# HyeonwooNoh/RAU_VQA

Measured on AMD Instinct MI355X. Metric: QA-pairs/sec fwd+bwd, Ours_SS 8-step RAU, batch 256, 14x14x512, higher is better.
Workload: dtype f32; 1 GPU; Ours_SS 8-step RAU fwd+bwd, 14x14x512, configs[1]; batch_per_gpu=256, global_batch=256, T=26, feature_map=14x14x512, hops=8, parallelism=dp1, collective=none, hop_weights=SS (x nHop), arithmetic=f32 operands, f32 MFMA accumulate, dropout=train mode, Philox masks per step and rank, launch=eager, 3 streams

## Files before the change

### rau_vqa_amd/csrc/gemm_conv.hip

```cpp
#include <cstdlib>

#include "gemm_core.h"
#include "kernels.h"

namespace rau {

constexpr int BK = 32;



static bool wide_on(int which) {
  static const int mask = [] { const char* e = std::getenv("RAU_CONV_WIDE"); return e ? std::atoi(e) : 3; }();
  return (mask & which) != 0;
}
static int wide_per_cu() {
  static const int v = [] { const char* e = std::getenv("RAU_CONV_WIDE_PER_CU"); return e ? std::atoi(e) : 1; }();
  return v == 2 ? 2 : 1;
}

hipError_t conv_embed_fwd(hipStream_t st, int nB, int D, int S, int M, const float* X,
                          const float* WiT, const float* bi, float* I, int bf16, int one_per_cu) {
  GemmParams P{};
  P.M = M; P.N = nB * S; P.K = D; P.nk = (D + BK - 1) / BK;
  P.A = WiT; P.a_rs = M;
  P.B = X; P.b_rs = S; P.b_bs = (long)D * S;
  P.S = S;
  P.C = I; P.c_bs = (long)M * S;
  P.bias = bi;
  P.act = 1;
  if (!bf16 && wide_on(1) && conv_wide_ok(M, D, S, M) && nB >= 4) {
    const int n4 = nB & ~3;
    hipError_t e = conv_wide(st, 0, n4, M, D, S, WiT, M, X, (long)D * S, I, (long)M * S, bi, 1, nullptr,
                             nullptr, nullptr, nullptr, 0, one_per_cu ? 1 : wide_per_cu());
    if (e != hipSuccess || n4 == nB) return e;
    return conv_embed_fwd(st, nB - n4, D, S, M, X + (size_t)n4 * D * S, WiT, bi, I + (size_t)n4 * M * S,
                          bf16, one_per_cu);
  }
  if (!bf16 && conv_sample_ok(S, 1))
    return conv_sample(st, 0, nB, M, D, S, WiT, M, X, (long)D * S, I, (long)M * S, bi, 1, nullptr, nullptr);
  if (bf16 == 2) return launch_gemm<128, 128, BK, SRC_RC, SRC_RC_FLAT, EPI_CONV, 2>(st, P, 1);
  if (bf16) return launch_gemm<128, 128, BK, SRC_RC, SRC_RC_FLAT, EPI_CONV, 1>(st, P, 1);
  return launch_gemm<128, 128, BK, SRC_RC, SRC_RC_FLAT, EPI_CONV>(st, P, 1, one_per_cu ? 30 * 1024 : 0);
}

static int b16_fwd_pad() { return 1024; }
hipError_t conv_embed_fwd_b16(hipStream_t st, int nB, int D, int S, int M, const void* X16,
                              const void* WiT16, const float* bi, float* I) {
  GemmParams P{};
  P.M = M; P.N = nB * S; P.K = D; P.nk = (D + BK - 1) / BK;
  P.A = reinterpret_cast<const float*>(WiT16); P.a_rs = M;
  P.B = reinterpret_cast<const float*>(X16); P.b_rs = S; P.b_bs = (long)D * S;
  P.S = S;
  P.C = I; P.c_bs = (long)M * S;
  P.bias = bi;
  P.act = 1;
  return launch_gemm<128, 128, BK, SRC_RC_B16, SRC_RC_FLAT_B16, EPI_CONV, 1>(st, P, 1, b16_fwd_pad());
}
hipError_t conv_att_pre_b16(hipStream_t st, int nB, int M, int S, int A, const float* I,
                            const void* WpT16, const float* bp, float* Pout) {
  GemmParams P{};
  P.M = A; P.N = nB * S; P.K = M; P.nk = (M + BK - 1) / BK;
  P.A = reinterpret_cast<const float*>(WpT16); P.a_rs = A;
  P.B = I; P.b_rs = S; P.b_bs = (long)M * S;
  P.S = S;
  P.C = Pout; P.c_bs = (long)A * S;
  P.bias = bp;
  P.act = 0;
  return launch_gemm<128, 128, BK, SRC_RC_B16, SRC_RC_FLAT, EPI_CONV, 1>(st, P, 1, b16_fwd_pad());
}

hipError_t conv_att_pre(hipStream_t st, int nB, int M, int S, int A, const float* I,
                        const float* WpT, const float* bp, float* Pout, int bf16, int one_per_cu) {
  GemmParams P{};
  P.M = A; P.N = nB * S; P.K = M; P.nk = (M + BK - 1) / BK;
  P.A = WpT; P.a_rs = A;
  P.B = I; P.b_rs = S; P.b_bs = (long)M * S;
  P.S = S;
  P.C = Pout; P.c_bs = (long)A * S;
  P.bias = bp;
  P.act = 0;
  if (!bf16 && wide_on(2) && conv_wide_ok(A, M, S, A) && nB >= 4) {
    const int n4 = nB & ~3;
    hipError_t e = conv_wide(st, 0, n4, A, M, S, WpT, A, I, (long)M * S, Pout, (long)A * S, bp, 0, nullptr,
                             nullptr, nullptr, nullptr, 0, one_per_cu ? 1 : wide_per_cu());
    if (e != hipSuccess || n4 == nB) return e;
    return conv_att_pre(st, nB - n4, M, S, A, I + (size_t)n4 * M * S, WpT, bp, Pout + (size_t)n4 * A * S,
                        bf16, one_per_cu);
  }
  if (!bf16 && conv_sample_ok(S, 2))
    return conv_sample(st, 0, nB, A, M, S, WpT, A, I, (long)M * S, Pout, (long)A * S, bp, 0, nullptr, nullptr);
  if (bf16 == 2) return launch_gemm<128, 128, BK, SRC_RC, SRC_RC_FLAT, EPI_CONV, 2>(st, P, 1);
  if (bf16) return launch_gemm<128, 128, BK, SRC_RC, SRC_RC_FLAT, EPI_CONV, 1>(st, P, 1);
  return launch_gemm<128, 128, BK, SRC_RC, SRC_RC_FLAT, EPI_CONV>(st, P, 1, one_per_cu ? 30 * 1024 : 0);
}

hipError_t conv_att_dgrad(hipStream_t st, int nB, int M, int S, int A, const float* dS,
                          const float* Wp, const float* dj, const float* a, float* dI, int bf16) {
  GemmParams P{};
  P.M = M; P.N = nB * S; P.K = A; P.nk = (A + BK - 1) / BK;
  P.A = Wp; P.a_rs = M;
  P.B = dS; P.b_rs = S; P.b_bs = (long)A * S;
  P.S = S;
  P.C = dI; P.c_bs = (long)M * S;
  P.v1 = dj; P.v2 = a;
  if (bf16 != 2 && M % 4 == 0 && conv_sample_ok(S, 4))
    return conv_sample(st, 1, nB, M, A, S, Wp, M, dS, (long)A * S, dI, (long)M * S, nullptr, 0, dj, a);
  if (bf16 == 2) return launch_gemm<128, 128, BK, SRC_RC, SRC_RC_FLAT, EPI_OUTER, 2>(st, P, 1);
  if (bf16) return launch_gemm<128, 128, BK, SRC_RC, SRC_RC_FLAT, EPI_OUTER, 1>(st, P, 1);
  return launch_gemm<128, 128, BK, SRC_RC, SRC_RC_FLAT, EPI_OUTER>(st, P, 1);
}

bool conv_dz_fused_ok(int S, int M, int bf16) {
  return bf16 != 2 && M % 4 == 0 && conv_sample_ok(S, 4);
}
hipError_t conv_att_dgrad_dz(hipStream_t st, int nB, int M, int S, int A, const float* dS,
                             const float* Wp, const float* dj, const float* a, const float* I,
                             float* dZ, float* rs, int dz16, int bf16, int ds16, int light) {
  if (bf16 == 1 && dgrad16_ok(M, A, S, M))
    return dgrad16(st, nB, M, A, S, Wp, M, dS, (long)A * S, dZ, (long)M * S, dj, a, I, rs, dz16, ds16);
  if (ds16) return hipErrorInvalidValue;
  if (!dz16 && !light && dgrad_dma_ok(M, A, S, M))
    return dgrad_dma(st, nB, M, A, S, Wp, M, dS, (long)A * S, dZ, (long)M * S, dj, a, I, rs);
  return conv_sample(st, 2, nB, M, A, S, Wp, M, dS, (long)A * S, dZ, (long)M * S, nullptr, 0, dj, a, I, rs,
                     dz16);
}

hipError_t conv_embed_dgrad(hipStream_t st, int nB, int D, int S, int M, const float* dZ,
                            const float* Wi, float* dX) {
  GemmParams P{};
  P.M = D; P.N = nB * S; P.K = M; P.nk = (M + BK - 1) / BK;
  P.A = Wi; P.a_rs = D;
  P.B = dZ; P.b_rs = S; P.b_bs = (long)M * S;
  P.S = S;
  P.C = dX; P.c_bs = (long)D * S;
  P.bias = nullptr;
  P.act = 0;
  if (conv_sample_ok(S, 8))
    return conv_sample(st, 0, nB, D, M, S, Wi, D, dZ, (long)M * S, dX, (long)D * S, nullptr, 0, nullptr, nullptr);
  return launch_gemm<128, 128, BK, SRC_RC, SRC_RC_FLAT, EPI_CONV>(st, P, 1);
}

static int conv_wgrad_splits(int nB, int rowsA, int rowsB) {
  const int tiles = ((rowsA + 127) / 128) * ((rowsB + 127) / 128);
  constexpr int target = 512;
  int s = target / tiles;
  if (s > nB) s = nB;
  if (s < 1) s = 1;
  return s;
}
size_t conv_wgrad_slab_floats(int nB, int rowsA, int rowsB, int S) {
  return (size_t)conv_wgrad_splits(nB, rowsA, rowsB) * ((size_t)rowsA * rowsB + rowsA);
}

template <int BKT, int ASRC, int DT = 0, int BSRC = SRC_SC>
static hipError_t conv_wgrad(hipStream_t st, GemmParams P, int nB, int S, float* dW,
                             float* slab, float* drow = nullptr) {
  P.S = S;
  P.cps = (S + BKT - 1) / BKT;
  P.K = S;
  P.nk = nB * P.cps;
  const int s = conv_wgrad_splits(nB, P.M, P.N);
  const int spb = (nB + s - 1) / s;
  P.C = slab; P.c_rs = P.N; P.slab_stride = (long)P.M * P.N;
  P.tiles_m = (P.M + 127) / 128;
  P.tiles_n = (P.N + 127) / 128;
  P.nk_per_split = spb * P.cps;
  const int splits = (P.nk + P.nk_per_split - 1) / P.nk_per_split;
  P.rs_out = drow ? slab + (size_t)splits * P.M * P.N : nullptr;
  {
    dim3 grid(8 * ((splits + 7) / 8) * P.tiles_m * P.tiles_n);
    hipLaunchKernelGGL((gemm_split_xcd_kernel<128, 128, BKT, ASRC, BSRC, EPI_SLAB, DT>), grid,
                       dim3(256), 0, st, P, splits);
  }
  hipError_t e = hipGetLastError();
  if (e != hipSuccess) return e;
  e = splitk_reduce_acc(st, (size_t)P.M * P.N, splits, slab, (size_t)P.M * P.N, dW);
  if (e != hipSuccess || !drow) return e;
  return splitk_reduce_acc(st, (size_t)P.M, splits, P.rs_out, (size_t)P.M, drow);
}
template <int ASRC>
static hipError_t conv_wgrad_any(hipStream_t st, const GemmParams& P, int nB, int S, float* dW,
                                 float* slab, int bf16, float* drow = nullptr) {
  if (!bf16 && ASRC == SRC_SC && !drow && wgrad_dma_ok(P.M, P.N, S))
    return wgrad_dma(st, nB, P.M, P.N, S, P.A, P.a_bs, P.B, P.b_bs, dW, slab, conv_wgrad_splits(nB, P.M, P.N));
  if (bf16 == 2) return conv_wgrad<32, ASRC, 2>(st, P, nB, S, dW, slab, drow);
  if (bf16) return conv_wgrad<32, ASRC, 1>(st, P, nB, S, dW, slab, drow);
  if (S % 28 == 0) return conv_wgrad<28, ASRC>(st, P, nB, S, dW, slab, drow);
  return conv_wgrad<32, ASRC>(st, P, nB, S, dW, slab, drow);
}

hipError_t conv_att_wgrad(hipStream_t st, int nB, int M, int S, int A, const float* dS,
                          const float* I, float* dWp, float* slab, int bf16) {
  GemmParams P{};
  P.M = A; P.N = M;
  P.A = dS; P.a_bs = (long)A * S;
  P.B = I; P.b_bs = (long)M * S;
  return conv_wgrad_any<SRC_SC>(st, P, nB, S, dWp, slab, bf16);
}

hipError_t conv_att_wgrad_ds16(hipStream_t st, int nB, int M, int S, int A, const void* dS16,
                               const float* I, float* dWp, float* slab) {
  GemmParams P{};
  P.M = A; P.N = M;
  P.A = reinterpret_cast<const float*>(dS16); P.a_bs = (long)A * S;
  P.B = I; P.b_bs = (long)M * S;
  return conv_wgrad<32, SRC_SC_B16, 1, SRC_SC>(st, P, nB, S, dWp, slab);
}

hipError_t conv_embed_wgrad(hipStream_t st, int nB, int D, int S, int M, const float* dI,
                            const float* I, const float* X, float* dWi, float* slab, int bf16,
                            float* dbi, int dz_final) {
  GemmParams P{};
  P.M = M; P.N = D;
  P.A = dI; P.A2 = I; P.a_bs = (long)M * S;
  P.B = X; P.b_bs = (long)D * S;
  if (dz_final) return conv_wgrad_any<SRC_SC>(st, P, nB, S, dWi, slab, bf16);
  return conv_wgrad_any<SRC_SC_DTANH>(st, P, nB, S, dWi, slab, bf16, dbi);
}

hipError_t conv_embed_wgrad_b16(hipStream_t st, int nB, int D, int S, int M, const void* dZ16,
                                const void* X16, float* dWi, float* slab) {
  if (wgrad16_ok(M, D, S))
    return wgrad16(st, nB, M, D, S, dZ16, (long)M * S, X16, (long)D * S, dWi, slab);
  GemmParams P{};
  P.M = M; P.N = D;
  P.A = reinterpret_cast<const float*>(dZ16); P.a_bs = (long)M * S;
  P.B = reinterpret_cast<const float*>(X16); P.b_bs = (long)D * S;
  return conv_wgrad<32, SRC_SC_B16, 1, SRC_SC_B16>(st, P, nB, S, dWi, slab);
}

}
```

### rau_vqa_amd/csrc/kernels.h

```cpp
#pragma once
#include <hip/hip_runtime.h>
#include <stddef.h>
#include <stdint.h>

#include "../../include/rau.h"

namespace rau {

constexpr long kMaxSplits = 4096;
constexpr hipError_t kSplitStateError = hipErrorIllegalState;
void split_ws_register(const float* base, size_t floats);
void split_ws_unregister(const float* base);
bool split_span_ok(const float* slab, long nsplit, size_t per_split_floats);

struct LinOpts {
  const float* bias = nullptr;
  const float* bias2 = nullptr;
  const float* addend = nullptr;
  long add_rs = 0;
  int accumulate = 0;
  int act = 0;
  const float* ymul = nullptr;
  long y_rs = 0;
  const uint32_t* emask = nullptr;
  size_t emask_e0 = 0;
  float emscale = 1.f;
  float alpha = 1.f;
  float* slab = nullptr;
  size_t slab_floats = 0;
  int* defer_splits = nullptr;
};
hipError_t gemm_nt(hipStream_t st, int M, int N, int K, const float* A, long lda,
                   const float* W, long ldw, float* C, long ldc, const LinOpts& o);
hipError_t gemm_nn(hipStream_t st, int M, int N, int K, const float* A, long lda,
                   const float* W, long ldw, float* C, long ldc, const LinOpts& o);
hipError_t gemm_nt_batched_deferred(hipStream_t st, int nb, int M, int N, int K,
                                    const float* const* A, long lda, const float* const* W,
                                    long ldw, float* slab, size_t slab_floats, int* splits);
hipError_t gemm_nn_batched_deferred(hipStream_t st, int nb, int M, int N, int K,
                                    const float* const* A, long lda, const float* const* W,
                                    long ldw, float* slab, size_t slab_floats, int* splits);
hipError_t gemm_nt_hetero_deferred(hipStream_t st, int nb, int M, int K, const float* A, long lda,
                                   const float* const* W, long ldw, const int* N, float* slab,
                                   size_t slab_floats, int* splits, size_t* off);
size_t gemm_tn_slab_floats(int M, int N, int K);
hipError_t gemm_tn_acc(hipStream_t st, int M, int N, int K, const float* A, long lda,
                       const float* B, long ldb, float* C, long ldc, float* slab,
                       float* dbias = nullptr, int bf16 = 0);

struct TnProblem {
  int M, N; const float* A; long lda; const float* B; long ldb; float* C; float* dbias;
};
size_t gemm_tn_group_slab_floats(const TnProblem* pr, int np, int K);
hipError_t gemm_tn_group_acc(hipStream_t st, const TnProblem* pr, int np, int K, float* slab,
                             size_t slab_floats, int bf16 = 0);

hipError_t conv_embed_fwd(hipStream_t st, int nB, int D, int S, int M, const float* X,
                          const float* WiT , const float* bi, float* I, int bf16 = 0,
                          int one_per_cu = 0 );
hipError_t conv_embed_fwd_b16(hipStream_t st, int nB, int D, int S, int M, const void* X16,
                              const void* WiT16, const float* bi, float* I);
hipError_t conv_att_pre_b16(hipStream_t st, int nB, int M, int S, int A, const float* I,
                            const void* WpT16, const float* bp, float* Pout);
hipError_t conv_att_pre(hipStream_t st, int nB, int M, int S, int A, const float* I,
                        const float* WpT , const float* bp, float* P, int bf16 = 0,
                        int one_per_cu = 0);
bool conv_sample_ok(int S, int which);
hipError_t conv_sample(hipStream_t st, int epi, int nB, int M, int K, int S, const float* Wt,
                       long w_rs, const float* X, long x_bs, float* C, long c_bs,
                       const float* bias, int act, const float* dj, const float* av,
                       const float* Y = nullptr, float* rs = nullptr, int c16 = 0);
bool conv_wide_ok(int M, int K, int S, long w_rs);
hipError_t conv_wide(hipStream_t st, int epi, int nB, int M, int K, int S, const float* Wt, long w_rs,
                     const float* X, long x_bs, float* C, long c_bs, const float* bias, int act,
                     const float* dj, const float* av, const float* Y, float* rs, int c16, int per_cu);
hipError_t transpose2d(hipStream_t st, int rows, int cols, const float* in, float* out,
                       void* out16 = nullptr);
hipError_t conv_att_dgrad(hipStream_t st, int nB, int M, int S, int A, const float* dS,
                          const float* Wp, const float* dj, const float* a, float* dI,
                          int bf16 = 0);
bool conv_dz_fused_ok(int S, int M, int bf16);
hipError_t conv_att_dgrad_dz(hipStream_t st, int nB, int M, int S, int A, const float* dS,
                             const float* Wp, const float* dj, const float* a, const float* I,
                             float* dZ, float* rs, int dz16 = 0,
                             int bf16 = 0,
                             int ds16 = 0,
                             int light = 0);
bool dgrad16_ok(int M, int K, int S, long w_rs);
hipError_t dgrad16(hipStream_t st, int nB, int M, int K, int S, const float* Wt, long w_rs,
                   const void* X, long x_bs, void* C, long c_bs, const float* dj, const float* av,
                   const float* Y, float* rs, int c16, int x16 = 0 );
bool dgrad_dma_ok(int M, int K, int S, long w_rs);
hipError_t dgrad_dma(hipStream_t st, int nB, int M, int K, int S, const float* Wt, long w_rs,
                     const float* X, long x_bs, float* C, long c_bs, const float* dj, const float* av,
                     const float* Y, float* rs);
hipError_t conv_att_wgrad_ds16(hipStream_t st, int nB, int M, int S, int A, const void* dS16,
                               const float* I, float* dWp, float* slab);
hipError_t conv_embed_dgrad(hipStream_t st, int nB, int D, int S, int M, const float* dZ,
                            const float* Wi, float* dX);
size_t conv_wgrad_slab_floats(int nB, int rowsA, int rowsB, int S);
bool wgrad16_ok(int ra, int rb, int S);
size_t wgrad16_slab_floats(int nB, int ra, int rb, int S);
hipError_t wgrad16(hipStream_t st, int nB, int ra, int rb, int S, const void* A16, long a_bs,
                   const void* B16, long b_bs, float* dW, float* slab);
bool skinny_dma_ok(int M, int K, long lda, long ldb, bool brc, int nprob, const int* N,
                   const float* const* A, const float* const* B);
int skinny_dma_splits(int M, int K, int tiles_all, size_t cols_all, size_t slab_floats);
void skinny_dma_set_deep(int on);
void lin_set_bf16(int on);
int lin_bf16();
hipError_t skinny_dma(hipStream_t st, bool brc, int nprob, int M, int K, const float* const* A,
                      long lda, const float* const* B, long ldb, const int* N, float* slab,
                      const long* off, int splits);
bool wgrad_dma_ok(int ra, int rb, int S);
hipError_t wgrad_dma(hipStream_t st, int nB, int ra, int rb, int S, const float* A, long a_bs,
                     const float* B, long b_bs, float* dW, float* slab, int splits);
hipError_t conv_att_wgrad(hipStream_t st, int nB, int M, int S, int A, const float* dS,
                          const float* I, float* dWp, float* slab, int bf16 = 0);
hipError_t conv_embed_wgrad(hipStream_t st, int nB, int D, int S, int M, const float* dI,
                            const float* I, const float* X, float* dWi, float* slab,
                            int bf16 = 0, float* dbi = nullptr ,
                            int dz_final = 0 );
hipError_t conv_embed_wgrad_b16(hipStream_t st, int nB, int D, int S, int M, const void* dZ16,
                                const void* X16, float* dWi, float* slab);

enum GateOrder { GATES_ATT = 0 ,
                 GATES_DEEP = 1  };

hipError_t fill_masks(hipStream_t st, uint64_t seed, uint32_t site, uint32_t step, float p,
                      size_t n, uint32_t* bits, const uint64_t* key_dev = nullptr);
hipError_t embed_fwd(hipStream_t st, int rows, int E, int V, const float* emb, const int32_t* tokens,
                     const uint32_t* mask, float mscale, float* we, size_t mask_e0 = 0);
hipError_t embed_bwd_rows(hipStream_t st, int rows, int E, int V, const int32_t* tokens, const float* dwe,
                          const float* we, const uint32_t* mask, size_t mask_e0, float mscale,
                          float* gE);
hipError_t lstm_fwd(hipStream_t st, int order, int nB, int R, float* g4, const float* c_prev,
                    long cp_rs, float* c, long c_rs, float* h, long h_rs, float* tanhc,
                    float* drop_out, const uint32_t* mask, size_t mask_e0, float mscale,
                    const float* slab = nullptr, int nsplit = 0);
hipError_t lstm_bwd(hipStream_t st, int order, int nB, int R, const float* gates,
                    const float* c_prev, long cp_rs, const float* tanhc, const float* dh,
                    long dh_rs, const float* dh2, const float* dc_next, float* dsum,
                    float* dc_prev, const int32_t* lens, int t, const float* dq_c,
                    const float* dq_h, long dq_rs, const float* slab = nullptr, int nsplit = 0);
struct LstmFwdCell {
  float* g4;
  int has_input;
  const float* b1; const float* b2;
  const float* slab; int nsplit;
  const float* c_prev; long cp_rs;
  float* c; long c_rs; float* h; long h_rs; float* tanhc;
  float* drop_out; const uint32_t* mask; size_t mask_e0; float mscale;
};
struct LstmFwdCells { int n; LstmFwdCell c[2]; };
hipError_t lstm_fwd_multi(hipStream_t st, int order, int nB, int R, const LstmFwdCells& cells);
struct EncWsParams {
  int B, R, TL, P;
  float *G1, *G2, *h1, *c1, *tc1, *x2, *h2, *c2, *tc2;
  const float *Wh1, *Wi2, *Wh2, *bi2, *bh2;
  const uint32_t* mask; float mscale;
  unsigned* cnt; int* err;
  int bf16 = 0;
};
bool enc_ws_ok(int B, int R);
int enc_ws_workgroups(int B);
bool enc_ws_coresident(int B, int blocks_per_cu, int n_cus);
bool enc_ws_fits_device(int B);
hipError_t enc_ws_forward(hipStream_t st, int order, EncWsParams Q);
struct LstmBwdCell {
  const float* gates; const float* c_prev; long cp_rs; const float* tanhc;
  const float* slabA; int nA;
  const float* slabB; int nBp;
  const uint32_t* maskB; size_t maskB_e0; float mscaleB;
  const float* dc_next; float* dsum; float* dc_prev;
  int t; const float* dq_c; const float* dq_h;
};
struct LstmBwdCells { int n; const int32_t* lens; long dq_rs; LstmBwdCell c[2]; };
hipError_t lstm_bwd_multi(hipStream_t st, int order, int nB, int R, const LstmBwdCells& cells);
struct AttPartials { int u_ns = 0; const float* u_bias = nullptr; int z_ns = 0; const float* z_bias = nullptr; int SL = 0; float* u_out = nullptr; int waves = 0;
                     const int32_t* img = nullptr; };
hipError_t att_fwd_fused(hipStream_t st, int nB, int M, int A, int S, const float* P,
                         const float* u, const float* ws, const float* bs, const float* zm,
                         const float* I, const float* qf, float* T, float* a, float* jv,
                         const AttPartials& ap = AttPartials());
hipError_t att_bwd_fused(hipStream_t st, int nB, int M, int A, int S, const float* I,
                         const float* dj, const float* a, const float* da_lin,
                         const float* ws, float* T_to_dS, float* dz, float* du, float* dwsp,
                         const float* Psrc = nullptr ,
                         const float* u = nullptr,
                         int da_ns = 0, int SL = 0, const float* da_add = nullptr,
                         void* dS16 = nullptr,
                         int waves_hint = 0 );
bool att_bwd_dma_ok(int M, int A, int S, int waves_hint = 0);
size_t att_split_part_floats(int nB, int S);
hipError_t att_fwd_split(hipStream_t st, int nB, int M, int A, int S, const float* P,
                         const float* u, const float* ws, const float* bs, const float* zm,
                         const float* I, const float* qf, float* a, float* jv, float* part,
                         const AttPartials& ap = AttPartials());
hipError_t att_bwd_split(hipStream_t st, int nB, int M, int A, int S, const float* I,
                         const float* dj, const float* a, const float* da_lin, const float* ws,
                         float* T_to_dS, float* dz, float* du, float* dwsp, const float* Psrc,
                         const float* u, float* part, int da_ns = 0, int SL = 0,
                         const float* da_add = nullptr);
inline bool feat_type_ok(int ft) { return ft == RAU_FEAT_F32 || ft == RAU_FEAT_F16 || ft == RAU_FEAT_BF16; }
hipError_t dropout_features(hipStream_t st, int H, size_t per_hop, const void* X,
                            const uint32_t* mask, float mscale, float* xd, size_t mask_e0 = 0,
                            int SL = 0, int Sp = 0, int ft = RAU_FEAT_F32);
hipError_t dropout_features_gen(hipStream_t st, uint64_t seed, uint32_t site, uint32_t step, float p,
                                const uint64_t* key_dev, int H, size_t per_hop, const void* X,
                                float mscale, void* xd, int b16, int ft = RAU_FEAT_F32);
hipError_t dropout_features_b16(hipStream_t st, int H, size_t per_hop, const void* X,
                                const uint32_t* mask, float mscale, void* xd16, int ft = RAU_FEAT_F32);
hipError_t widen_features(hipStream_t st, size_t rows, int SL, int Sp, const void* X, float* out, int ft);
hipError_t expand_features(hipStream_t st, int nB, size_t map_bytes, const void* table, const int32_t* image_of,
                           void* out);
hipError_t bank_gather(hipStream_t st, int n, size_t map_bytes, const void* bank, int32_t capacity,
                       const int32_t* rows, void* out);
hipError_t narrow_features(hipStream_t st, size_t rows, int SL, int Sp, const float* src, void* out, int ft);
hipError_t colsum_acc(hipStream_t st, int rows, int N, const float* X, long ld, float* dst,
                      float* tmp);
hipError_t ce_fwd(hipStream_t st, int nB, int K, int M, const float* logits,
                  const int32_t* labels, const float* mf, const float* wd, const float* bd,
                  float* dl, float* lossrow, int32_t* argmax, float* dopred,
                  const float* part = nullptr, int nsplit = 0, const float* bias = nullptr,
                  float* logits_out = nullptr,
                  int Bper = 0 );
hipError_t loss_reduce(hipStream_t st, int H, int nB, const float* lossrow, float* losses);
hipError_t scale_hops(hipStream_t st, int H, size_t per_hop, const float* w_dev, float* x);
hipError_t scale_hops3(hipStream_t st, int H, const float* w_dev, size_t p0, float* x0, size_t p1, float* x1,
                       size_t p2, float* x2);
hipError_t gather_q(hipStream_t st, int nB, int Rq, int T, const int32_t* lens, const float* c1,
                    const float* h1, const float* c2, const float* h2, float* q);
hipError_t apply_mask(hipStream_t st, size_t n, size_t period, const float* x,
                      const uint32_t* mask, float mscale, float* y, size_t mask_e0 = 0);
hipError_t row_scale(hipStream_t st, int rows, int N, const float* s, const float* X,
                     const float* v, float* out);
hipError_t sigmoid_bwd(hipStream_t st, int n, const float* dy, const float* y, float* dx);
hipError_t mul_dtanh(hipStream_t st, size_t n, const float* d, const float* y, float* out);
hipError_t scale_inplace(hipStream_t st, size_t n, float s, float* x);
hipError_t dq_reduce(hipStream_t st, int H, size_t n, const float* dQD, const uint32_t* mask,
                     float mscale, float* dq);
hipError_t embed_bwd(hipStream_t st, int nuniq, int E, const int32_t* utok, const int32_t* ustart,
                     const int32_t* upos, const float* dwe, const float* we,
                     const uint32_t* mask, float mscale, float* gE);
hipError_t splitk_reduce_acc(hipStream_t st, size_t n, int splits, const float* slab,
                             size_t slab_stride, float* dst);
hipError_t lin_reduce_epilogue(hipStream_t st, int M, int N, int splits, const float* slab,
                               float* C, long ldc, const LinOpts& o);
hipError_t uniform_fill(hipStream_t st, uint64_t seed, uint32_t stream, size_t n, float lo,
                        float hi, float* x);
hipError_t add_noise_sqnorm(hipStream_t st, size_t n, float* g, float nstd, uint64_t seed,
                            uint32_t stream, float* partial );
hipError_t finish_norm(hipStream_t st, int nparts, const float* partial, float* norm_out);
hipError_t clip_adam(hipStream_t st, size_t n, float* x, float* g, float* m, float* v,
                     const float* norm, float clip, float stepsize, float beta1, float beta2,
                     float eps);
hipError_t step_stats(hipStream_t st, int H, int B, int K, const float* logits, const float* dopred,
                      const int32_t* argmax, const float* lossrow, const int32_t* labels, float* rowf,
                      int32_t* rowi, float* out);
hipError_t predict_rows(hipStream_t st, int H, int B, int K, int Sp, const float* logits, const float* dopred,
                        const float* att, const int32_t* mc, int n_mc, int32_t* oe, int32_t* mco, float* pred,
                        float* att_out);
size_t predict_rows_lds(int K);

}
```

### rau_vqa_amd/csrc/kernels.hip

```cpp
#include "common.h"
#include <cstdlib>

#include "kernels.h"
#include "philox.h"

namespace rau {

static inline int grid_for(size_t n, int block = 256, int cap = 256 * 8) {
  size_t g = (n + block - 1) / block;
  if (g > (size_t)cap) g = cap;
  if (g < 1) g = 1;
  return (int)g;
}

__global__ void k_fill_masks(uint64_t seed, uint32_t site, uint32_t step, uint32_t thr,
                             size_t nwords, uint32_t* __restrict__ bits,
                             const uint64_t* __restrict__ key) {
  RAU_CHAIN_PRIO();
  if (key) {
    seed = key[0];
    step = (uint32_t)key[1];
  }
  for (size_t w = blockIdx.x * (size_t)blockDim.x + threadIdx.x; w < nwords;
       w += (size_t)gridDim.x * blockDim.x) {
// ... 1193 lines not shown
  __syncthreads();
  const int rows = (A + NC - 1) / NC, k_lo = c * rows, k_hi = min(A, k_lo + rows);
  float* Tb = T + (size_t)b * A * S;
  const float* Pb = Psrc ? Psrc + (size_t)b * A * S : nullptr;
  constexpr int UB = 2;
  for (int k0 = k_lo + w; k0 < k_hi; k0 += 4 * UB) {
    float s1[UB], s2[UB];
#pragma unroll
    for (int i = 0; i < UB; ++i) s1[i] = s2[i] = 0.f;
    for (int q = l; q < S4; q += 64) {
      const float4 d = reinterpret_cast<const float4*>(dzs)[q];
      float4 t[UB];
#pragma unroll
      for (int i = 0; i < UB; ++i) {
        const int k = k0 + 4 * i;
        t[i] = make_float4(0.f, 0.f, 0.f, 0.f);
        if (k < k_hi)
          t[i] = Psrc ? reinterpret_cast<const float4*>(Pb + (size_t)k * S)[q]
                      : reinterpret_cast<const float4*>(Tb + (size_t)k * S)[q];
      }
#pragma unroll
      for (int i = 0; i < UB; ++i) {
        const int k = k0 + 4 * i;
        if (k < k_hi) {
          const float wk = ws[k];
          if (Psrc) {
            const float uk = u[(size_t)b * A + k];
            t[i].x = tanh_fast(t[i].x + uk); t[i].y = tanh_fast(t[i].y + uk);
            t[i].z = tanh_fast(t[i].z + uk); t[i].w = tanh_fast(t[i].w + uk);
          }
          float4 o;
          o.x = d.x * wk * (1.f - t[i].x * t[i].x);
          o.y = d.y * wk * (1.f - t[i].y * t[i].y);
          o.z = d.z * wk * (1.f - t[i].z * t[i].z);
          o.w = d.w * wk * (1.f - t[i].w * t[i].w);
          reinterpret_cast<float4*>(Tb + (size_t)k * S)[q] = o;
          s1[i] += (o.x + o.y) + (o.z + o.w);
          s2[i] += d.x * t[i].x + d.y * t[i].y + d.z * t[i].z + d.w * t[i].w;
        }
      }
    }
#pragma unroll
    for (int i = 0; i < UB; ++i) {
      const int k = k0 + 4 * i;
      const float v1 = wave_sum(s1[i]);
      const float v2 = wave_sum(s2[i]);
      if (l == 0 && k < k_hi) {
        du[(size_t)b * A + k] = v1;
        dwsp[(size_t)b * A + k] = v2;
      }
    }
  }
}

hipError_t att_bwd_split(hipStream_t st, int nB, int M, int A, int S, const float* I,
                         const float* dj, const float* a, const float* da_lin, const float* ws,
                         float* T_to_dS, float* dz, float* du, float* dwsp, const float* Psrc,
                         const float* u, float* part, int da_ns, int SL, const float* da_add) {
  if (!split_span_ok(da_lin, da_ns, (size_t)nB * (SL ? SL : S))) return kSplitStateError;
  const int nc = att_chunks(nB);
  hipLaunchKernelGGL(k_att_da_part, dim3(nc, nB), dim3(256), (size_t)4 * S * sizeof(float), st, M, S, I,
                     dj, part);
  hipLaunchKernelGGL(k_att_ds, dim3(nc, nB), dim3(256), (size_t)(S + 4) * sizeof(float), st, nB, A, S,
                     part, a, da_lin, ws, T_to_dS, dz, du, dwsp, Psrc, u, da_ns, SL, da_add);
  return hipGetLastError();
}

__global__ void k_transpose2d(int rows, int cols, const float* __restrict__ in,
                              float* __restrict__ out, __bf16* __restrict__ out16) {
  __shared__ float tile[32][33];
  const int c0 = blockIdx.x * 32, r0 = blockIdx.y * 32;
  const int tx = threadIdx.x & 31, ty = threadIdx.x >> 5;
  for (int j = ty; j < 32; j += 8)
    if (r0 + j < rows && c0 + tx < cols) tile[j][tx] = in[(size_t)(r0 + j) * cols + c0 + tx];
  __syncthreads();
  for (int j = ty; j < 32; j += 8)
    if (c0 + j < cols && r0 + tx < rows) {
      out[(size_t)(c0 + j) * rows + r0 + tx] = tile[tx][j];
      if (out16) out16[(size_t)(c0 + j) * rows + r0 + tx] = (__bf16)tile[tx][j];
    }
}
hipError_t transpose2d(hipStream_t st, int rows, int cols, const float* in, float* out, void* out16) {
  hipLaunchKernelGGL(k_transpose2d, dim3((cols + 31) / 32, (rows + 31) / 32), dim3(256), 0, st,
                     rows, cols, in, out, reinterpret_cast<__bf16*>(out16));
  return hipGetLastError();
}

__device__ __forceinline__ float widen_f16(uint32_t h) {
  const uint32_t sign = (h & 0x8000u) << 16, e = (h >> 10) & 0x1fu, m = h & 0x3ffu;
  if (e == 0) {
    const float v = (float)m * 0x1p-24f;
    return __uint_as_float(__float_as_uint(v) | sign);
  }
  return __uint_as_float(sign | (e == 31 ? 0x7f800000u : (e + 112u) << 23) | (m << 13));
}
template <int FT>
__device__ __forceinline__ float widen1(uint32_t h) {
  return FT == RAU_FEAT_F16 ? widen_f16(h) : __uint_as_float(h << 16);
}
template <int FT>
__device__ __forceinline__ float load_feat(const void* __restrict__ X, size_t i) {
  if (FT == RAU_FEAT_F32) return reinterpret_cast<const float*>(X)[i];
  return widen1<FT>(reinterpret_cast<const uint16_t*>(X)[i]);
}
template <int FT>
__device__ __forceinline__ float4 load_feat4(const void* __restrict__ X, size_t q) {
  if (FT == RAU_FEAT_F32) return reinterpret_cast<const float4*>(X)[q];
  const uint2 v = reinterpret_cast<const uint2*>(X)[q];
  return make_float4(widen1<FT>(v.x & 0xffffu), widen1<FT>(v.x >> 16), widen1<FT>(v.y & 0xffffu),
                     widen1<FT>(v.y >> 16));
}

template <int FT>
__global__ void k_dropout_features(int H, size_t per4, const void* __restrict__ X,
                                   const uint32_t* __restrict__ mask, size_t e0, float mscale,
                                   float4* __restrict__ xd) {
  for (size_t q = blockIdx.x * (size_t)blockDim.x + threadIdx.x; q < per4;
       q += (size_t)gridDim.x * blockDim.x) {
    const float4 x = load_feat4<FT>(X, q);
    for (int h = 0; h < H; ++h) {
      const size_t e = e0 + ((size_t)h * per4 + q) * 4;
      const uint32_t nib = mask_nib(mask, e);
      float4 o;
      o.x = (nib & 1u) ? x.x * mscale : 0.f;
      o.y = (nib & 2u) ? x.y * mscale : 0.f;
      o.z = (nib & 4u) ? x.z * mscale : 0.f;
      o.w = (nib & 8u) ? x.w * mscale : 0.f;
      xd[(size_t)h * per4 + q] = o;
    }
  }
}
template <int FT>
__global__ void k_dropout_features_b16(int H, size_t per4, const void* __restrict__ X,
                                       const uint32_t* __restrict__ mask, size_t e0, float mscale,
                                       uint2* __restrict__ xd) {
  for (size_t q = blockIdx.x * (size_t)blockDim.x + threadIdx.x; q < per4;
       q += (size_t)gridDim.x * blockDim.x) {
    const float4 x = load_feat4<FT>(X, q);
    for (int h = 0; h < H; ++h) {
      const size_t e = e0 + ((size_t)h * per4 + q) * 4;
      const uint32_t nib = mask_nib(mask, e);
      typedef __bf16 b16x4 __attribute__((ext_vector_type(4)));
      b16x4 o;
      o[0] = (__bf16)((nib & 1u) ? x.x * mscale : 0.f);
      o[1] = (__bf16)((nib & 2u) ? x.y * mscale : 0.f);
      o[2] = (__bf16)((nib & 4u) ? x.z * mscale : 0.f);
      o[3] = (__bf16)((nib & 8u) ? x.w * mscale : 0.f);
      xd[(size_t)h * per4 + q] = __builtin_bit_cast(uint2, o);
    }
  }
}
template <bool B16, int FT>
__global__ void k_dropout_features_gen(uint64_t seed, uint32_t site, uint32_t step, uint32_t thr,
                                       const uint64_t* __restrict__ key, int H, size_t per16,
                                       const void* __restrict__ X, float mscale,
                                       void* __restrict__ xd) {
  if (key) {
    seed = key[0];
    step = (uint32_t)key[1];
  }
  const int l = threadIdx.x & 63, quad = l & 3, sub = l >> 2;
  for (size_t base = (blockIdx.x * (size_t)blockDim.x + (threadIdx.x & ~63u)); base < per16;
       base += (size_t)gridDim.x * blockDim.x) {
    float4 x[4];
    bool ok[4];
#pragma unroll
    for (int r = 0; r < 4; ++r) {
      const size_t blk = base + 16 * r + sub;
      ok[r] = blk < per16;
      x[r] = ok[r] ? load_feat4<FT>(X, 4 * blk + quad) : make_float4(0.f, 0.f, 0.f, 0.f);
    }
    const size_t mine = base + l < per16 ? base + l : per16 - 1;
    for (int h = 0; h < H; ++h) {
      const uint32_t bits = philox_keep16(seed, site, step, (size_t)h * per16 + mine, thr);
#pragma unroll
      for (int r = 0; r < 4; ++r) {
        const uint32_t nib = (uint32_t)__shfl((int)bits, 16 * r + sub, 64) >> (4 * quad);
        float4 o;
        o.x = (nib & 1u) ? x[r].x * mscale : 0.f;
        o.y = (nib & 2u) ? x[r].y * mscale : 0.f;
        o.z = (nib & 4u) ? x[r].z * mscale : 0.f;
        o.w = (nib & 8u) ? x[r].w * mscale : 0.f;
        const size_t q = ((size_t)h * per16 + base + 16 * r + sub) * 4 + quad;
        if (!ok[r]) continue;
        if (B16) {
          typedef __bf16 b16x4 __attribute__((ext_vector_type(4)));
          b16x4 v;
          v[0] = (__bf16)o.x; v[1] = (__bf16)o.y; v[2] = (__bf16)o.z; v[3] = (__bf16)o.w;
          reinterpret_cast<uint2*>(xd)[q] = __builtin_bit_cast(uint2, v);
        } else {
          reinterpret_cast<float4*>(xd)[q] = o;
        }
      }
    }
  }
}
template <bool B16>
static void launch_dropout_gen(hipStream_t st, int ft, dim3 grid, uint64_t seed, uint32_t site,
                               uint32_t step, uint32_t thr, const uint64_t* key, int H, size_t per16,
                               const void* X, float mscale, void* xd) {
  if (ft == RAU_FEAT_F16)
    hipLaunchKernelGGL((k_dropout_features_gen<B16, RAU_FEAT_F16>), grid, dim3(256), 0, st, seed, site, step,
                       thr, key, H, per16, X, mscale, xd);
  else if (ft == RAU_FEAT_BF16)
    hipLaunchKernelGGL((k_dropout_features_gen<B16, RAU_FEAT_BF16>), grid, dim3(256), 0, st, seed, site, step,
                       thr, key, H, per16, X, mscale, xd);
  else
    hipLaunchKernelGGL((k_dropout_features_gen<B16, RAU_FEAT_F32>), grid, dim3(256), 0, st, seed, site, step,
                       thr, key, H, per16, X, mscale, xd);
}
hipError_t dropout_features_gen(hipStream_t st, uint64_t seed, uint32_t site, uint32_t step, float p,
                                const uint64_t* key_dev, int H, size_t per_hop, const void* X,
                                float mscale, void* xd, int b16, int ft) {
  if (per_hop % 16 != 0 || !feat_type_ok(ft)) return hipErrorInvalidValue;
  const uint32_t thr = (uint32_t)lroundf(p * 256.0f);
  const size_t per16 = per_hop / 16;
  if (b16)
    launch_dropout_gen<true>(st, ft, dim3(grid_for(per16)), seed, site, step, thr, key_dev, H, per16, X,
                             mscale, xd);
  else
    launch_dropout_gen<false>(st, ft, dim3(grid_for(per16)), seed, site, step, thr, key_dev, H, per16, X,
                              mscale, xd);
  return hipGetLastError();
}
template <int FT>
__global__ void k_dropout_features_pitch(int H, size_t rows, int SL, int Sp,
                                         const void* __restrict__ X,
                                         const uint32_t* __restrict__ mask, size_t e0, float mscale,
                                         float* __restrict__ xd) {
  const size_t n = rows * Sp;
  for (size_t i = blockIdx.x * (size_t)blockDim.x + threadIdx.x; i < n;
       i += (size_t)gridDim.x * blockDim.x) {
    const size_t r = i / Sp;
    const int s = (int)(i - r * Sp);
    const float x = load_feat<FT>(X, i);
    for (int h = 0; h < H; ++h) {
      float o = 0.f;
      if (s < SL) o = mask_bit(mask, e0 + ((size_t)h * rows + r) * SL + s) ? x * mscale : 0.f;
      xd[(size_t)h * n + i] = o;
    }
  }
}
#define LAUNCH_FT(kern, ft, grid, ...)                                                        \
  do {                                                                                        \
    if ((ft) == RAU_FEAT_F16)                                                                 \
      hipLaunchKernelGGL(kern<RAU_FEAT_F16>, grid, dim3(256), 0, st, __VA_ARGS__);            \
    else if ((ft) == RAU_FEAT_BF16)                                                           \
      hipLaunchKernelGGL(kern<RAU_FEAT_BF16>, grid, dim3(256), 0, st, __VA_ARGS__);           \
    else                                                                                      \
      hipLaunchKernelGGL(kern<RAU_FEAT_F32>, grid, dim3(256), 0, st, __VA_ARGS__);            \
  } while (0)
hipError_t dropout_features(hipStream_t st, int H, size_t per_hop, const void* X,
                            const uint32_t* mask, float mscale, float* xd, size_t mask_e0, int SL,
                            int Sp, int ft) {
  if (!feat_type_ok(ft)) return hipErrorInvalidValue;
  if (SL != Sp) {
    LAUNCH_FT(k_dropout_features_pitch, ft, dim3(grid_for(per_hop)), H, per_hop / Sp, SL, Sp, X, mask,
              mask_e0, mscale, xd);
    return hipGetLastError();
  }
  LAUNCH_FT(k_dropout_features, ft, dim3(grid_for(per_hop / 4)), H, per_hop / 4, X, mask, mask_e0, mscale,
            reinterpret_cast<float4*>(xd));
  return hipGetLastError();
}

hipError_t dropout_features_b16(hipStream_t st, int H, size_t per_hop, const void* X,
                                const uint32_t* mask, float mscale, void* xd16, int ft) {
  if (!feat_type_ok(ft)) return hipErrorInvalidValue;
  LAUNCH_FT(k_dropout_features_b16, ft, dim3(grid_for(per_hop / 4)), H, per_hop / 4, X, mask, (size_t)0,
            mscale, reinterpret_cast<uint2*>(xd16));
  return hipGetLastError();
}

template <int FT>
__global__ void k_widen_features(size_t per4, const void* __restrict__ X, float4* __restrict__ out) {
  for (size_t q = blockIdx.x * (size_t)blockDim.x + threadIdx.x; q < per4;
       q += (size_t)gridDim.x * blockDim.x)
    out[q] = load_feat4<FT>(X, q);
}
template <int FT>
__global__ void k_widen_features_pitch(size_t rows, int SL, int Sp, const void* __restrict__ X,
                                       float* __restrict__ out) {
  const size_t n = rows * Sp;
  for (size_t i = blockIdx.x * (size_t)blockDim.x + threadIdx.x; i < n;
       i += (size_t)gridDim.x * blockDim.x) {
    const size_t r = i / Sp;
    const int s = (int)(i - r * Sp);
    out[i] = s < SL ? load_feat<FT>(X, i) : 0.f;
  }
}
hipError_t widen_features(hipStream_t st, size_t rows, int SL, int Sp, const void* X, float* out, int ft) {
  if (ft != RAU_FEAT_F16 && ft != RAU_FEAT_BF16) return hipErrorInvalidValue;
  if (SL != Sp) {
    LAUNCH_FT(k_widen_features_pitch, ft, dim3(grid_for(rows * Sp)), rows, SL, Sp, X, out);
    return hipGetLastError();
  }
  if ((rows * Sp) % 4 != 0) return hipErrorInvalidValue;
  LAUNCH_FT(k_widen_features, ft, dim3(grid_for(rows * Sp / 4)), rows * Sp / 4, X,
            reinterpret_cast<float4*>(out));
  return hipGetLastError();
}
#undef LAUNCH_FT

template <typename V>
__global__ __launch_bounds__(256) void k_expand_features(size_t nvec, const V* __restrict__ table,
                                                         const int32_t* __restrict__ image_of,
                                                         V* __restrict__ out) {
  const int b = blockIdx.y;
  const int ib = __builtin_amdgcn_readfirstlane(image_of[b]);
  const V* src = table + (size_t)ib * nvec;
  V* dst = out + (size_t)b * nvec;
  for (size_t i = blockIdx.x * (size_t)blockDim.x + threadIdx.x; i < nvec; i += (size_t)gridDim.x * blockDim.x)
    dst[i] = src[i];
}
hipError_t expand_features(hipStream_t st, int nB, size_t map_bytes, const void* table, const int32_t* image_of,
                           void* out) {
  if (nB <= 0 || !table || !image_of || !out || map_bytes % 8 != 0) return hipErrorInvalidValue;
  const bool v16 = map_bytes % 16 == 0;
  const size_t nvec = map_bytes / (v16 ? 16 : 8);
  const int slices = (int)std::min<size_t>(16, (nvec + 1023) / 1024);
  const dim3 grid(std::max(slices, 1), nB);
  if (v16)
    hipLaunchKernelGGL(k_expand_features<uint4>, grid, dim3(256), 0, st, nvec, static_cast<const uint4*>(table),
                       image_of, static_cast<uint4*>(out));
  else
    hipLaunchKernelGGL(k_expand_features<uint2>, grid, dim3(256), 0, st, nvec, static_cast<const uint2*>(table),
                       image_of, static_cast<uint2*>(out));
  return hipGetLastError();
}

constexpr int kColChunks = 32;
__global__ void k_colsum_stage1(int rows, int N, const float* __restrict__ X, long ld,
                                float* __restrict__ tmp) {
  RAU_CHAIN_PRIO();
  const int n = blockIdx.x * blockDim.x + threadIdx.x;
  if (n >= N) return;
  const int per = (rows + kColChunks - 1) / kColChunks;
  const int r0 = blockIdx.y * per;
  int r1 = r0 + per;
  if (r1 > rows) r1 = rows;
  float acc = 0.f;
  for (int r = r0; r < r1; ++r) acc += X[(size_t)r * ld + n];
  tmp[(size_t)blockIdx.y * N + n] = acc;
}
__global__ __launch_bounds__(256) void k_colsum_stage1_v4(int rows, int N,
                                                         const float* __restrict__ X, long ld,
                                                         float* __restrict__ tmp) {
  __shared__ float4 part[4][64];
  const int l = threadIdx.x & 63, w = threadIdx.x >> 6;
  const int n = (blockIdx.x * 64 + l) * 4;
  const int per = (rows + kColChunks - 1) / kColChunks;
  const int r0 = blockIdx.y * per;
  int r1 = r0 + per;
  if (r1 > rows) r1 = rows;
  float4 a0 = make_float4(0.f, 0.f, 0.f, 0.f), a1 = a0, a2 = a0, a3 = a0;
  if (n < N) {
    const float* p = X + n;
    int r = r0 + w;
    for (; r + 12 < r1; r += 16) {
      const float4 x0 = *reinterpret_cast<const float4*>(p + (size_t)r * ld);
      const float4 x1 = *reinterpret_cast<const float4*>(p + (size_t)(r + 4) * ld);
      const float4 x2 = *reinterpret_cast<const float4*>(p + (size_t)(r + 8) * ld);
      const float4 x3 = *reinterpret_cast<const float4*>(p + (size_t)(r + 12) * ld);
      a0.x += x0.x; a0.y += x0.y; a0.z += x0.z; a0.w += x0.w;
      a1.x += x1.x; a1.y += x1.y; a1.z += x1.z; a1.w += x1.w;
      a2.x += x2.x; a2.y += x2.y; a2.z += x2.z; a2.w += x2.w;
      a3.x += x3.x; a3.y += x3.y; a3.z += x3.z; a3.w += x3.w;
    }
    for (; r < r1; r += 4) {
      const float4 x0 = *reinterpret_cast<const float4*>(p + (size_t)r * ld);
      a0.x += x0.x; a0.y += x0.y; a0.z += x0.z; a0.w += x0.w;
    }
  }
  float4 a;
// ... 437 lines not shown
```

### rau_vqa_amd/csrc/rau_ctx.h

```cpp
#pragma once
#include <hip/hip_runtime.h>

#include <algorithm>
#include <cmath>
#include <cstdarg>
#include <cstdio>
#include <cstdlib>
#include <cstring>
#include <numeric>
#include <string>
#include <vector>

#include "../../include/rau.h"
#include "kernels.h"

using namespace rau;

constexpr int kEncHeadTokens = 4;
constexpr int kEncSideChunks = 4;
#define LINOPTS(name) LinOpts name; name.slab = ctx->slab; name.slab_floats = ctx->slab_floats

__attribute__((visibility("hidden"))) int fail(int code, const char* fmt, ...);
#define HIPC(expr)                                                                        \
  do {                                                                                    \
    hipError_t e_ = (expr);                                                               \
    if (e_ != hipSuccess)                                                                 \
      return fail(RAU_ERR_DEVICE, "%s failed: %s (%s:%d)", #expr, hipGetErrorString(e_),  \
                  __FILE__, __LINE__);                                                    \
  } while (0)
#define NEED(cond, ...)                               \
  do {                                                \
    if (!(cond)) return fail(RAU_ERR_INVALID, __VA_ARGS__); \
  } while (0)

struct Lin {
  float *W, *b, *dW, *db;
  int out, in;
};
struct Entry {
  std::string name;
  size_t off;
  int rows, cols;
};
struct Group {
  float* w = nullptr;
  float* g = nullptr;
  float* m = nullptr;
  float* v = nullptr;
  size_t n = 0;
  int64_t adam_t = 0;
  std::vector<Entry> layout;
};
struct ProfRec {
  int cls;
  hipEvent_t a, b;
  int sid;
};
struct ProfCls {
  std::string name;
  int64_t launches = 0;
  double ms = 0, flops = 0, bytes = 0;
};

struct BatchDesc {
  int feat_type = RAU_FEAT_F32;
  int n_images = 0;
  bool bank = false;
  bool table_ok = false;
  std::vector<int32_t> lens;
  int max_len = 0, nuniq = 0;
  bool have = false, have_labels = false;
};
struct BatchSlot {
  float* feats = nullptr;
  int32_t *tokens = nullptr, *lens_d = nullptr, *labels_d = nullptr;
  int32_t *utok = nullptr, *ustart = nullptr, *upos = nullptr;
  int32_t* image_of_d = nullptr;
  int32_t* bank_idx_d = nullptr;
  float* feats_h = nullptr;
  int32_t *tokens_h = nullptr, *lens_p = nullptr, *labels_h = nullptr;
  int32_t *utok_h = nullptr, *ustart_h = nullptr, *upos_h = nullptr;
  int32_t* image_of_h = nullptr;
  int32_t* bank_idx_h = nullptr;
  hipEvent_t uploaded = nullptr;
  hipEvent_t consumed = nullptr;
  BatchDesc held;
  bool upload_pending = false, consumed_valid = false;
};

struct rau_ctx {
  rau_config cfg;
  int cap = 0;
  int Q;
  int Sp = 0;
  int bf16 = 0;
  hipStream_t st = nullptr;
  hipStream_t st2 = nullptr;
  hipStream_t st3 = nullptr;
  hipEvent_t evA = nullptr, evD = nullptr, evW = nullptr, evE = nullptr, evW3 = nullptr,
             evM3 = nullptr, evEnd = nullptr, evE1 = nullptr, evHd = nullptr,
             evG0 = nullptr, evG = nullptr, evQ0 = nullptr, evQ = nullptr, evDq = nullptr;
  hipEvent_t evGc[kEncSideChunks] = {};
  int enc_chunk_tok[kEncSideChunks + 1] = {};
  std::vector<hipEvent_t> evH;
  std::vector<hipEvent_t> evF, evK;
  std::vector<int> groups, cur, bgroups;
  std::vector<void*> allocs;
  std::vector<std::pair<void*, size_t>> scratch;
  Group grp[3];
  Lin q_proj, h_proj, i_embed, att_q, att_i, att_score, att_mem, feat_attprob, lstm_i2h,
      lstm_h2h, lstm_out, cls, do_pred;
  Lin i2h[2], h2h[2];
  float* feats_x = nullptr;
  bool x_valid = false;
  int x_slot = 0;
  uint64_t x_serial = 0;
  bool fwd_table = false;
  float* xw = nullptr;
  void* bank = nullptr;
  int32_t bank_cap = 0, bank_filled = 0;
  int bank_type = RAU_FEAT_F32;
  std::vector<uint8_t> bank_written;
  void* bank_pin[2] = {nullptr, nullptr};
  float* bank_stage = nullptr;
  size_t bank_chunk = 0;
  hipEvent_t bank_ev[2] = {nullptr, nullptr};
  BatchSlot slot[2];
  uint64_t slot_serial[2] = {0, 0};
  int cur_slot = 0;
  bool async_ready = false;
  hipStream_t stc = nullptr;
  hipEvent_t hopw_ev[2] = {nullptr, nullptr};
  int mode = RAU_MODE_TRAIN;
  uint32_t* mbits[5] = {nullptr, nullptr, nullptr, nullptr, nullptr};
  size_t mcount[5] = {0, 0, 0, 0, 0};
  bool mexplicit[5] = {false, false, false, false, false};
  float mp[5];
  float mp_exact[5];
  uint64_t seed = 0;
  uint32_t step = 0;
  float *we, *G1, *G2, *c1, *h1, *c2, *h2, *tc1, *tc2, *x2, *q;
  float *xd;
  void* WiT16 = nullptr;
  void* WpT16 = nullptr;
  void* dS16 = nullptr;
  bool dpre_fwd = false;
  bool ds16_step = false;
  void* xd16 = nullptr;
  bool I_shared = false;
  bool yq_shared = false;
  float *WiT, *WpT;
  float *P0;
  float *qd, *Yq, *qf, *I, *T, *u, *zm, *a, *jv, *j, *g4, *cc, *hh, *tc, *mf, *logits,
      *dl, *lossrow, *dopred, *losses_d, *hopw_d;
  int32_t* argmax_d;
  float* att_part = nullptr;
  bool att_split_env = false;
  bool enc_ws = false;
  bool enc_ws_train = false;
  int side_split_env = -1;
  unsigned* ws_cnt = nullptr;
  int* perr_d = nullptr;
  int* perr_h = nullptr;
  bool persist_used = false;
  bool persist_gave_up = false;
  float* hopw_h = nullptr;
  int hopw_slot = 0;
  float *dpre, *dhn, *dg4, *dcn[2], *dhp[2], *dj, *da_lin, *dz, *du, *dwsp, *dZ,
      *dqt, *dQD, *dq, *slab, *slab2, *slab3, *coltmp3, *tmpS, *coltmp2, *dbi_part;
  size_t slab3_floats = 0, slab2_floats = 0;
  size_t slab_alloc = 0, slab2_alloc = 0, slab3_alloc = 0;
  float *dG1, *dG2, *dwe, *edc[2][2];
  size_t slab_floats = 0;
  bool mod_ready = false;
  float *m_state = nullptr, *m_dstate = nullptr;
  float *m_tmp[4] = {nullptr, nullptr, nullptr, nullptr};
  float *m_dq = nullptr, *m_dc = nullptr, *m_dh = nullptr;
  float *m_Xp = nullptr, *m_a = nullptr, *m_da = nullptr, *m_dXd = nullptr;
  float* m_Xw = nullptr;
  float *m_dX = nullptr, *m_dZ = nullptr;
  float *m_add = nullptr, *m_s = nullptr, *m_zero = nullptr;
  float *m_loss = nullptr;
  uint64_t mod_masks_seed = 0;
  uint32_t mod_masks_step = 0;
  bool mod_masks_valid = false;
  void* comm = nullptr;
  hipStream_t st_comm = nullptr;
  hipEvent_t evC = nullptr;
  int comm_ranks = 0;
  uint64_t* dkey = nullptr;
  bool capturing = false;
  bool graph_last = false;
  std::vector<std::pair<uint64_t, hipGraphExec_t>> graphs;
  bool mg_valid = false;
  bool mg_labels = false;
  const int32_t* mg_labels_d = nullptr;
  int mg_slot = 0;
  uint64_t mg_serial = 0;
  bool mg_ready = false, mg_merged = false;
  float *mg_rowf = nullptr, *mg_out = nullptr, *mg_pred = nullptr, *mg_att = nullptr;
  int32_t *mg_rowi = nullptr, *mg_ans = nullptr, *mg_mc = nullptr;
  size_t mg_mc_cap = 0;
  float *npart = nullptr, *norms_d = nullptr;
  bool fwd_done = false, bwd_done = false;
  hipEvent_t ev0 = nullptr, ev1 = nullptr;
  bool prof_on = false;
  bool prof_sparse = false;
  std::vector<ProfCls> pcls;
  std::vector<ProfRec> precs;
  std::vector<hipEvent_t> evpool;
};

inline BatchSlot& cur_batch(rau_ctx* ctx) { return ctx->slot[ctx->cur_slot]; }
inline const BatchSlot& cur_batch(const rau_ctx* ctx) { return ctx->slot[ctx->cur_slot]; }

inline bool chain_bound(const rau_ctx* ctx) {
  return ctx->mode == RAU_MODE_EVAL || ctx->bf16 || ctx->cfg.B <= 64;
}
inline bool side_split(const rau_ctx* ctx) {
  if (ctx->side_split_env >= 0) return ctx->side_split_env != 0;
  return chain_bound(ctx);
}
inline void set_skinny_policy(const rau_ctx* ctx) {
  static const int env = [] { const char* e = std::getenv("RAU_SKINNY_DEEP"); return e ? (std::atoi(e) != 0 ? 1 : 0) : -1; }();
  skinny_dma_set_deep(env >= 0 ? env : (chain_bound(ctx) ? 1 : 0));
  lin_set_bf16(ctx->bf16 == 1);
}
inline void merge_record(rau_ctx* ctx) {
  ctx->mg_valid = true;
  ctx->mg_labels = cur_batch(ctx).held.have_labels;
  ctx->mg_labels_d = cur_batch(ctx).labels_d;
  ctx->mg_slot = ctx->cur_slot;
  ctx->mg_serial = ctx->slot_serial[ctx->cur_slot];
}
inline float mask_p(const rau_ctx* ctx, int site) {
  return ctx->mexplicit[site] ? ctx->mp_exact[site] : ctx->mp[site];
}

template <typename Tp>
static int dalloc(rau_ctx* c, Tp** p, size_t count, bool scratch = true) {
  void* d = nullptr;
  const size_t bytes = std::max<size_t>(count, 1) * sizeof(Tp);
  hipError_t e = hipMalloc(&d, bytes);
  if (e != hipSuccess)
    return fail(RAU_ERR_NOMEM, "hipMalloc(%zu bytes) failed: %s", bytes, hipGetErrorString(e));
  e = hipMemsetAsync(d, 0, bytes, c->st);
  if (e != hipSuccess) return fail(RAU_ERR_DEVICE, "hipMemsetAsync: %s", hipGetErrorString(e));
  c->allocs.push_back(d);
  if (scratch) c->scratch.push_back({d, bytes});
  *p = reinterpret_cast<Tp*>(d);
  return 0;
}

struct LayoutBuilder {
  Group* g;
  size_t off = 0;
  Lin take(const char* name, int out, int in) {
    Lin l;
    l.out = out;
    l.in = in;
    g->layout.push_back({std::string(name) + ".weight", off, out, in});
    l.W = reinterpret_cast<float*>(off);
    off += (size_t)out * in;
    g->layout.push_back({std::string(name) + ".bias", off, out, 1});
    l.b = reinterpret_cast<float*>(off);
    off += out;
    return l;
  }
};
static inline void bind(Lin& l, const Group& g) {
  const size_t ow = reinterpret_cast<size_t>(l.W), ob = reinterpret_cast<size_t>(l.b);
  l.W = g.w + ow;
  l.b = g.w + ob;
  l.dW = g.g + ow;
  l.db = g.g + ob;
}

static inline int prof_class(rau_ctx* c, const char* name) {
  for (size_t i = 0; i < c->pcls.size(); ++i)
    if (c->pcls[i].name == name) return (int)i;
  c->pcls.push_back(ProfCls{name});
  return (int)c->pcls.size() - 1;
}
static inline hipEvent_t prof_event(rau_ctx* c) {
  if (!c->evpool.empty()) {
    hipEvent_t e = c->evpool.back();
    c->evpool.pop_back();
    return e;
  }
  hipEvent_t e;
  hipEventCreate(&e);
  return e;
}

static inline bool prof_marker(const char* n) {
  for (const char* m : {"embed_fwd", "gather_q", "loss_reduce", "scale_hops", "dq_reduce", "embed_bwd"})
    if (std::strcmp(n, m) == 0) return true;
  return false;
}
#ifdef RAU_DEV_HOOKS
static inline bool rau_dev_skipped(const char* cname) {
  static const std::string list = [] { const char* e = std::getenv("RAU_DEV_SKIP"); return std::string(e ? e : ""); }();
  if (list.empty()) return false;
  size_t pos = 0;
  const std::string n(cname);
  while (pos <= list.size()) {
    const size_t c = list.find(',', pos);
    const std::string tok = list.substr(pos, c == std::string::npos ? std::string::npos : c - pos);
    if (tok == n) return true;
    if (c == std::string::npos) break;
    pos = c + 1;
  }
  return false;
}
#define RAU_DEV_SKIPPED(cname) rau_dev_skipped(cname)
#else
#define RAU_DEV_SKIPPED(cname) false
#endif
#define RUN(cname, fl, by, expr) RUNS(ctx->st, cname, fl, by, expr)
#define RUNS(rstream, cname, fl, by, expr)                                                \
  do {                                                                                    \
    ProfRec pr_;                                                                          \
    int pc_ = -1;                                                                         \
// ... 53 lines not shown
```

### rau_vqa_amd/csrc/rau_ctx.hip

```cpp
#include "rau_ctx.h"

static thread_local char g_err[512] = "";
int fail(int code, const char* fmt, ...) {
  va_list ap;
  va_start(ap, fmt);
  vsnprintf(g_err, sizeof(g_err), fmt, ap);
  va_end(ap);
  return code;
}

static int prof_collect(rau_ctx* ctx) {
  if (ctx->precs.empty()) return 0;
  HIPC(hipStreamSynchronize(ctx->st));
  HIPC(hipStreamSynchronize(ctx->st2));
  HIPC(hipStreamSynchronize(ctx->st3));
  if (ctx->stc) HIPC(hipStreamSynchronize(ctx->stc));
  FILE* tl = nullptr;
  if (const char* p = std::getenv("RAU_PROF_TIMELINE")) tl = std::fopen(p, "a");
  for (auto& r : ctx->precs) {
    float ms = 0.f;
    hipEventElapsedTime(&ms, r.a, r.b);
    if (tl) {
      float t0 = 0.f;
      hipEventElapsedTime(&t0, ctx->precs[0].a, r.a);
      std::fprintf(tl, "%s,%d,%.4f,%.4f\n", ctx->pcls[r.cls].name.c_str(), r.sid, t0, t0 + ms);
    }
    ctx->pcls[r.cls].ms += ms;
    ctx->evpool.push_back(r.a);
    ctx->evpool.push_back(r.b);
  }
  ctx->precs.clear();
  if (tl) { std::fprintf(tl, "#\n"); std::fclose(tl); }
  return 0;
}
static int mult_wgrad_problems(rau_ctx* ctx, TnProblem* pr) {
  const rau_config& c = ctx->cfg;
  const int S = ctx->Sp, SL = c.S, M = c.M, A = c.A, R = c.R, K = c.K, Q = ctx->Q;
  const size_t BR_ = (size_t)c.B * R;
  const float* hprev = ctx->hh;
  const float* hnew = ctx->hh + BR_;
  struct WG { Lin* l; const float* dY; long ldy; const float* X; long ldx; };
  const WG wgs[] = {
      {&ctx->cls, ctx->dl, K, ctx->mf, M},             {&ctx->lstm_out, ctx->dpre, M, hnew, R},
      {&ctx->lstm_i2h, ctx->dg4, 4 * R, ctx->j, M},    {&ctx->lstm_h2h, ctx->dg4, 4 * R, hprev, R},
      {&ctx->feat_attprob, ctx->dj, M, ctx->a, S},     {&ctx->att_mem, ctx->dz, S, hprev, R},
      {&ctx->att_q, ctx->du, A, ctx->qf, M},           {&ctx->q_proj, ctx->dqt, M, ctx->qd, Q},
      {&ctx->h_proj, ctx->dqt, M, hprev, R}};
  int n = 0;
  for (const WG& w : wgs) {
    const int out = w.l == &ctx->att_mem ? SL : w.l->out;
    const int in = w.l == &ctx->feat_attprob ? SL : w.l->in;
    pr[n++] = TnProblem{out, in, w.dY, w.ldy, w.X, w.ldx, w.l->dW, w.l->db};
  }
  return n;
}
static int enc_wgrad_problems(rau_ctx* ctx, size_t row0, TnProblem* pr) {
  struct WG { Lin* l; const float* dY; const float* X; };
  const WG wgs[] = {{&ctx->i2h[0], ctx->dG1, ctx->we}, {&ctx->h2h[0], ctx->dG1, ctx->h1},
                    {&ctx->i2h[1], ctx->dG2, ctx->x2}, {&ctx->h2h[1], ctx->dG2, ctx->h2}};
  int n = 0;
  for (const WG& w : wgs)
    pr[n++] = TnProblem{w.l->out, w.l->in, w.dY + row0 * w.l->out, w.l->out,
                        w.X + row0 * w.l->in, w.l->in, w.l->dW, w.l->db};
  return n;
}

struct BatchPlan {
  std::vector<int> groups;
  bool att_split, enc_ws, enc_ws_train;
  size_t slab, slab2, slab3, att_part;
  size_t mcount[5];
};
static void plan_batch(rau_ctx* ctx, int B, BatchPlan* p) {
  const rau_config& c = ctx->cfg;
  const int T = c.T, E = c.E, Rq = c.Rq, D = c.D, S = ctx->Sp, SL = c.S, M = c.M, A = c.A, R = c.R, K = c.K,
            H = c.H, Q = ctx->Q;
  {
    std::vector<int> sizes;
    if (const char* eg = std::getenv("RAU_HOP_GROUPS")) {
      int sum = 0;
      for (const char* q = eg; *q;) {
        const int v = std::atoi(q);
        if (v < 1) { sizes.clear(); break; }
        sizes.push_back(v);
        sum += v;
        while (*q && *q != ',') ++q;
        if (*q == ',') ++q;
      }
      if (sum != H) sizes.clear();
    }
    if (sizes.empty() && B <= 64) {
      sizes.push_back(H);
    }
    if (sizes.empty()) {
      int left = H;
      while (left > 3) { sizes.push_back(2); left -= 2; }
      while (left > 0) { sizes.push_back(1); left -= 1; }
      if (H == 2) sizes = {1, 1};
    }
    p->groups.assign(H, 0);
    int h0 = 0;
    for (int n : sizes) { p->groups[h0] = n; h0 += n; }
  }
  p->mcount[RAU_MASK_WE] = (size_t)T * B * E;
  p->mcount[RAU_MASK_RNN] = (size_t)T * B * Rq;
  p->mcount[RAU_MASK_Q] = (size_t)H * B * Q;
  p->mcount[RAU_MASK_X] = (size_t)H * B * D * SL;
  p->mcount[RAU_MASK_MF] = (size_t)H * B * M;
  p->att_part = att_split_part_floats(B, S);
  p->att_split = std::getenv("RAU_ATT_SPLIT") != nullptr ||
                 (B <= 64 && std::getenv("RAU_ATT_FUSED") == nullptr);
  {
    const char* e = std::getenv("RAU_ENC_WS");
    const bool fits = !ctx->persist_gave_up && enc_ws_ok(B, Rq) && enc_ws_fits_device(B);
    p->enc_ws_train = fits && (e ? std::atoi(e) != 0 : B <= 32);
    p->enc_ws = fits && (e ? std::atoi(e) != 0 : B <= 64);
  }
  {
    size_t sl2 = std::max(conv_wgrad_slab_floats(H * B, A, M, S),
                          conv_wgrad_slab_floats(H * B, M, D, S));
    if (ctx->bf16) sl2 = std::max(sl2, wgrad16_slab_floats(H * B, M, D, S));
    size_t grp_floats = 0;
    {
      TnProblem pr[13];
      int n = mult_wgrad_problems(ctx, pr);
      for (int hh = 1; hh <= H; ++hh)
        grp_floats = std::max(grp_floats, gemm_tn_group_slab_floats(pr, n, hh * B));
      n = enc_wgrad_problems(ctx, 0, pr);
      for (int tt = 1; tt <= T; ++tt)
        grp_floats = std::max(grp_floats, gemm_tn_group_slab_floats(pr, n, tt * B));
    }
    p->slab2 = std::max(sl2, grp_floats);
    const int rowsH = H * B, rowsT = T * B;
    const int shapes[][3] = {{K, M, rowsH},      {M, R, rowsH},      {4 * R, M, rowsH},
                             {4 * R, R, rowsH},  {M, S, rowsH},      {S, R, rowsH},
                             {A, M, rowsH},      {M, Q, rowsH},      {4 * Rq, E, rowsT},
                             {4 * Rq, Rq, rowsT}};
    size_t sl = (size_t)16 * B * std::max({4 * R, 4 * Rq, K, Q, M, A, S});
    for (auto& sh : shapes) sl = std::max(sl, gemm_tn_slab_floats(sh[0], sh[1], sh[2]));
    p->slab = sl;
    p->slab3 = std::max(sl, grp_floats);
  }
}
static void adopt_plan(rau_ctx* ctx, const BatchPlan& p) {
  ctx->groups = p.groups;
  for (int i = 0; i < 5; ++i) ctx->mcount[i] = p.mcount[i];
  ctx->att_split_env = p.att_split;
  ctx->enc_ws = p.enc_ws;
  ctx->enc_ws_train = p.enc_ws_train;
  ctx->slab_floats = p.slab;
  ctx->slab2_floats = p.slab2;
  ctx->slab3_floats = p.slab3;
}

extern "C" {

const char* rau_last_error(void) { return g_err; }
int rau_abi_version(void) { return RAU_ABI_VERSION; }

int rau_split_guard_check(size_t ws_floats, size_t offset, int nsplit, size_t per_split_floats) {
  static thread_local float anchor[1];
  const float* base = anchor;
  split_ws_register(base, ws_floats);
  const bool ok = split_span_ok(base + offset, nsplit, per_split_floats);
  split_ws_unregister(base);
  if (!ok)
    return fail(RAU_ERR_STATE, "split-K partials [%zu + %d x %zu) outside a workspace of %zu floats: "
                               "nothing would be launched", offset, nsplit, per_split_floats, ws_floats);
  return RAU_OK;
}
int rau_enc_ws_coresident(int batch, int blocks_per_cu, int n_cus) {
  return (enc_ws_ok(batch, 512) && enc_ws_coresident(batch, blocks_per_cu, n_cus)) ? 1 : 0;
}

void rau_default_config(rau_config* cfg) {
  std::memset(cfg, 0, sizeof(*cfg));
  cfg->B = 100;
  cfg->T = 26;
  cfg->V = 14000;
  cfg->E = 200;
  cfg->Rq = 512;
  cfg->D = 512;
  cfg->S = 196;
  cfg->M = 512;
  cfg->A = 256;
  cfg->R = 512;
  cfg->K = 1000;
  cfg->H = 8;
  cfg->p_we = cfg->p_rnn = cfg->p_q = cfg->p_x = cfg->p_mf = 0.5f;
  cfg->dtype = RAU_F32;
  cfg->device_id = 0;
}

int rau_create(const rau_config* cfg, rau_ctx** out) {
  NEED(cfg && out, "rau_create: null argument");
  const rau_config& c = *cfg;
  NEED(c.B > 0 && c.T > 0 && c.V > 1 && c.H > 0, "rau_create: B,T,H must be > 0 and V > 1");
  NEED(c.E > 0 && c.E % 4 == 0, "rau_create: E=%d must be a positive multiple of 4", c.E);
  NEED(c.S > 0, "rau_create: S=%d must be positive", c.S);
  NEED(c.K > 0 && c.K % 4 == 0, "rau_create: K=%d must be a positive multiple of 4", c.K);
  NEED(c.Rq > 0 && c.Rq % 4 == 0 && c.R > 0 && c.R % 4 == 0 && c.M > 0 && c.M % 4 == 0 &&
           c.A > 0 && c.A % 4 == 0 && c.D > 0 && c.D % 4 == 0,
       "rau_create: Rq,R,M,A,D must be positive multiples of 4");
  NEED(c.dtype == RAU_F32 || c.dtype == RAU_BF16 || c.dtype == RAU_F32S,
       "rau_create: dtype %d not supported", c.dtype);
  const float ps[5] = {c.p_we, c.p_rnn, c.p_q, c.p_x, c.p_mf};
  for (float p : ps) NEED(p >= 0.f && p < 1.f, "rau_create: dropout p=%f out of [0,1)", p);

  int ndev = 0;
  hipError_t e = hipGetDeviceCount(&ndev);
  if (e != hipSuccess || ndev <= 0)
    return fail(RAU_ERR_DEVICE, "no HIP device available (%s); librau has no CPU fallback",
                hipGetErrorString(e));
  NEED(c.device_id >= 0 && c.device_id < ndev, "rau_create: device_id %d of %d", c.device_id, ndev);
  HIPC(hipSetDevice(c.device_id));
  hipDeviceProp_t prop;
  HIPC(hipGetDeviceProperties(&prop, c.device_id));
  if (std::strncmp(prop.gcnArchName, "gfx950", 6) != 0)
    return fail(RAU_ERR_DEVICE, "device %d is %s; librau is built for gfx950 only", c.device_id,
                prop.gcnArchName);

  rau_ctx* ctx = new rau_ctx();
  ctx->cfg = c;
  ctx->Q = 4 * c.Rq;
  ctx->Sp = (c.S + 3) & ~3;
  ctx->bf16 = c.dtype;
  for (int i = 0; i < 5; ++i) {
    const float pq = std::lround(ps[i] * 256.0f) / 256.0f;
    if (pq >= 1.f) {
      delete ctx;
      return fail(RAU_ERR_INVALID, "rau_create: dropout p=%f rounds to 1 at 1/256 resolution", ps[i]);
    }
    ctx->mp[i] = pq;
    ctx->mp_exact[i] = ps[i];
  }
  *out = nullptr;
#define CK(x)                \
  do {                       \
    int rc_ = (x);           \
    if (rc_ != 0) {          \
      rau_destroy(ctx);      \
      return rc_;            \
    }                        \
  } while (0)
  {
    int prio_lo = 0, prio_hi = 0;
    hipDeviceGetStreamPriorityRange(&prio_lo, &prio_hi);
    hipError_t es = hipStreamCreateWithPriority(&ctx->st, hipStreamNonBlocking, prio_hi);
    if (es == hipSuccess) es = hipStreamCreateWithPriority(&ctx->st2, hipStreamNonBlocking, prio_lo);
    if (es != hipSuccess) {
      delete ctx;
      return fail(RAU_ERR_DEVICE, "hipStreamCreate: %s", hipGetErrorString(es));
    }
  }
  hipEventCreate(&ctx->ev0);
  hipEventCreate(&ctx->ev1);
  const unsigned evflags = hipEventDisableTiming;
  for (hipEvent_t* e : {&ctx->evA, &ctx->evD, &ctx->evW, &ctx->evE, &ctx->evW3, &ctx->evM3, &ctx->evEnd, &ctx->evE1,
                        &ctx->evG0, &ctx->evG, &ctx->evQ0, &ctx->evQ, &ctx->evDq})
    hipEventCreateWithFlags(e, evflags);
  for (hipEvent_t& e : ctx->evGc) hipEventCreateWithFlags(&e, evflags);
  {
    int plo = 0, phi = 0;
    hipDeviceGetStreamPriorityRange(&plo, &phi);
    hipStreamCreateWithPriority(&ctx->st3, hipStreamNonBlocking, plo);
  }
  ctx->cap = c.B;
  {
    if (const char* eg = std::getenv("RAU_BWD_GROUPS")) {
      std::vector<int> bs;
      int sum = 0;
      for (const char* p = eg; *p;) {
        const int v = std::atoi(p);
        if (v < 1) { bs.clear(); sum = -1; break; }
        bs.push_back(v);
        sum += v;
        while (*p && *p != ',') ++p;
        if (*p == ',') ++p;
      }
      if (sum == c.H) {
        ctx->bgroups.assign(c.H, 0);
        int b0 = 0;
        for (int n : bs) { ctx->bgroups[b0] = n; b0 += n; }
      }
    }
  }
  ctx->evF.resize(c.H);
  ctx->evK.resize(c.H);

  ctx->evH.resize(c.H);
  for (int i = 0; i < c.H; ++i) {
    hipEventCreateWithFlags(&ctx->evF[i], evflags);
    hipEventCreateWithFlags(&ctx->evK[i], evflags);

    hipEventCreateWithFlags(&ctx->evH[i], evflags);
  }
  hipEventCreateWithFlags(&ctx->evHd, evflags);

  const int B = c.B, T = c.T, E = c.E, Rq = c.Rq, D = c.D, S = ctx->Sp, SL = c.S, M = c.M, A = c.A,
            R = c.R, K = c.K, H = c.H, Q = ctx->Q;
  {
    Group& g = ctx->grp[RAU_GROUP_EMBED];
    g.layout.push_back({"word_embed.weight", 0, c.V, E});
    g.n = (size_t)c.V * E;
  }
  {
    LayoutBuilder lb{&ctx->grp[RAU_GROUP_RNN]};
    ctx->i2h[0] = lb.take("rnn.l1.i2h", 4 * Rq, E);
    ctx->h2h[0] = lb.take("rnn.l1.h2h", 4 * Rq, Rq);
    ctx->i2h[1] = lb.take("rnn.l2.i2h", 4 * Rq, Rq);
    ctx->h2h[1] = lb.take("rnn.l2.h2h", 4 * Rq, Rq);
    ctx->grp[RAU_GROUP_RNN].n = lb.off;
  }
  {
    LayoutBuilder lb{&ctx->grp[RAU_GROUP_MULT]};
    ctx->q_proj = lb.take("q_embed.q_proj", M, Q);
    ctx->h_proj = lb.take("q_embed.h_proj", M, R);
    ctx->i_embed = lb.take("i_embed.conv", M, D);
    ctx->att_q = lb.take("attbycontent.qfeatatt", A, M);
    ctx->att_i = lb.take("attbycontent.ifeatproj", A, M);
    ctx->att_score = lb.take("attbycontent.attscore", 1, A);
    ctx->att_mem = lb.take("attbymemory.linear", SL, R);
    ctx->feat_attprob = lb.take("classifier.feat_attprob", M, SL);
    ctx->lstm_i2h = lb.take("classifier.attlstm.i2h", 4 * R, M);
    ctx->lstm_h2h = lb.take("classifier.attlstm.h2h", 4 * R, R);
    ctx->lstm_out = lb.take("classifier.lstm_out", M, R);
    ctx->cls = lb.take("classifier.out_score", K, M);
    ctx->do_pred = lb.take("classifier.out_do_pred", 1, M);
    ctx->grp[RAU_GROUP_MULT].n = lb.off;
  }
  for (int gi = 0; gi < 3; ++gi) {
    CK(dalloc(ctx, &ctx->grp[gi].w, ctx->grp[gi].n + 4, false));
    CK(dalloc(ctx, &ctx->grp[gi].g, ctx->grp[gi].n + 4, false));
  }
  for (int L = 0; L < 2; ++L) {
    bind(ctx->i2h[L], ctx->grp[RAU_GROUP_RNN]);
    bind(ctx->h2h[L], ctx->grp[RAU_GROUP_RNN]);
  }
  Lin* ml[] = {&ctx->q_proj, &ctx->h_proj, &ctx->i_embed, &ctx->att_q, &ctx->att_i,
               &ctx->att_score, &ctx->att_mem, &ctx->feat_attprob, &ctx->lstm_i2h,
               &ctx->lstm_h2h, &ctx->lstm_out, &ctx->cls, &ctx->do_pred};
  for (Lin* l : ml) bind(*l, ctx->grp[RAU_GROUP_MULT]);

  BatchPlan plan;
  plan_batch(ctx, B, &plan);
  adopt_plan(ctx, plan);
  BatchSlot& s0 = ctx->slot[0];
  CK(dalloc(ctx, &s0.feats, (size_t)B * D * S));
  CK(dalloc(ctx, &s0.tokens, (size_t)T * B));
  CK(dalloc(ctx, &s0.lens_d, (size_t)B));
  CK(dalloc(ctx, &s0.labels_d, (size_t)B));
  CK(dalloc(ctx, &s0.utok, (size_t)T * B));
  CK(dalloc(ctx, &s0.ustart, (size_t)T * B + 1));
  CK(dalloc(ctx, &s0.upos, (size_t)T * B));
  for (int i = 0; i < 5; ++i) CK(dalloc(ctx, &ctx->mbits[i], (ctx->mcount[i] + 31) / 32 + 1));
  const size_t TB = (size_t)T * B;
  CK(dalloc(ctx, &ctx->we, TB * E));
  CK(dalloc(ctx, &ctx->G1, TB * 4 * Rq));
  CK(dalloc(ctx, &ctx->G2, TB * 4 * Rq));
  CK(dalloc(ctx, &ctx->c1, (TB + B) * Rq));
  CK(dalloc(ctx, &ctx->h1, (TB + B) * Rq));
  CK(dalloc(ctx, &ctx->c2, (TB + B) * Rq));
  CK(dalloc(ctx, &ctx->h2, (TB + B) * Rq));
  CK(dalloc(ctx, &ctx->tc1, TB * Rq));
  CK(dalloc(ctx, &ctx->tc2, TB * Rq));
  CK(dalloc(ctx, &ctx->x2, TB * Rq));
  CK(dalloc(ctx, &ctx->q, (size_t)B * Q));
  const size_t HB = (size_t)H * B;
  CK(dalloc(ctx, &ctx->qd, HB * Q));
  CK(dalloc(ctx, &ctx->Yq, HB * M));
  CK(dalloc(ctx, &ctx->qf, HB * M));
  CK(dalloc(ctx, &ctx->xd, HB * D * S));
  if (ctx->bf16 == 1 && ctx->Sp == c.S && conv_dz_fused_ok(S, M, 1) && !std::getenv("RAU_XD_F32")) {
    float* x16 = nullptr;
    CK(dalloc(ctx, &x16, (HB * D * S + 1) / 2));
    ctx->xd16 = x16;
    float *w16 = nullptr, *p16 = nullptr;
    CK(dalloc(ctx, &w16, ((size_t)M * D + 1) / 2));
    CK(dalloc(ctx, &p16, ((size_t)A * M + 1) / 2));
    ctx->WiT16 = w16;
    ctx->WpT16 = p16;
    if (dgrad16_ok(M, A, S, M) && att_bwd_dma_ok(M, A, S, 8)) {
      float* d16 = nullptr;
      CK(dalloc(ctx, &d16, (HB * A * S + 1) / 2));
      ctx->dS16 = d16;
    }
  }
  CK(dalloc(ctx, &ctx->I, HB * M * S));
  CK(dalloc(ctx, &ctx->T, HB * A * S));
  CK(dalloc(ctx, &ctx->u, HB * A));
  CK(dalloc(ctx, &ctx->P0, (size_t)B * A * S));
  CK(dalloc(ctx, &ctx->WiT, (size_t)M * D));
  CK(dalloc(ctx, &ctx->WpT, (size_t)A * M));
  CK(dalloc(ctx, &ctx->zm, (size_t)B * S));
  CK(dalloc(ctx, &ctx->att_part, plan.att_part));
  {
    if (const char* ss = std::getenv("RAU_SIDE_SPLIT")) ctx->side_split_env = std::atoi(ss) != 0;
    float* f = nullptr;
    CK(dalloc(ctx, &f, 16));
    ctx->ws_cnt = reinterpret_cast<unsigned*>(f);
  }
  {
    float* f = nullptr;
    CK(dalloc(ctx, &f, 4));
    ctx->perr_d = reinterpret_cast<int*>(f);
    if (hipHostMalloc(reinterpret_cast<void**>(&ctx->perr_h), sizeof(int), hipHostMallocDefault) != hipSuccess)
      ctx->perr_h = nullptr;
    else
      *ctx->perr_h = 0;
  }
  CK(dalloc(ctx, &ctx->a, HB * S));
  CK(dalloc(ctx, &ctx->jv, (size_t)B * M));
  CK(dalloc(ctx, &ctx->j, HB * M));
  CK(dalloc(ctx, &ctx->g4, HB * 4 * R));
  CK(dalloc(ctx, &ctx->cc, (HB + B) * R));
  CK(dalloc(ctx, &ctx->hh, (HB + B) * R));
  CK(dalloc(ctx, &ctx->tc, HB * R));
  CK(dalloc(ctx, &ctx->mf, HB * M));
  CK(dalloc(ctx, &ctx->logits, HB * K));
  CK(dalloc(ctx, &ctx->dl, HB * K));
  CK(dalloc(ctx, &ctx->lossrow, HB));
  CK(dalloc(ctx, &ctx->dopred, HB));
  CK(dalloc(ctx, &ctx->losses_d, (size_t)H));
  CK(dalloc(ctx, &ctx->hopw_d, (size_t)H));
  {
    hipError_t eh = hipHostMalloc((void**)&ctx->hopw_h, (size_t)2 * H * sizeof(float), hipHostMallocDefault);
    if (eh != hipSuccess) {
      rau_destroy(ctx);
      return fail(RAU_ERR_NOMEM, "hipHostMalloc(hop weights): %s", hipGetErrorString(eh));
    }
  }
  CK(dalloc(ctx, &ctx->argmax_d, HB));
  CK(dalloc(ctx, &ctx->dpre, HB * M));
  CK(dalloc(ctx, &ctx->dhn, HB * R));
  CK(dalloc(ctx, &ctx->dg4, HB * 4 * R));
  for (int i = 0; i < 2; ++i) {
    CK(dalloc(ctx, &ctx->dcn[i], (size_t)B * R));
    CK(dalloc(ctx, &ctx->dhp[i], (size_t)B * R));
  }
  CK(dalloc(ctx, &ctx->dj, HB * M));
  CK(dalloc(ctx, &ctx->da_lin, (size_t)B * S));
  CK(dalloc(ctx, &ctx->dz, HB * S));
  CK(dalloc(ctx, &ctx->du, HB * A));
  CK(dalloc(ctx, &ctx->dwsp, HB * A));
  CK(dalloc(ctx, &ctx->dZ, HB * M * S));
  CK(dalloc(ctx, &ctx->dqt, HB * M));
  CK(dalloc(ctx, &ctx->dQD, HB * Q));
  CK(dalloc(ctx, &ctx->dq, (size_t)B * Q));
  {
    CK(dalloc(ctx, &ctx->slab2, plan.slab2));
    CK(dalloc(ctx, &ctx->slab, plan.slab));
    CK(dalloc(ctx, &ctx->slab3, plan.slab3));
    ctx->slab_alloc = plan.slab;
    ctx->slab2_alloc = plan.slab2;
    ctx->slab3_alloc = plan.slab3;
    split_ws_register(ctx->slab, ctx->slab_floats);
    split_ws_register(ctx->slab2, ctx->slab2_floats);
    split_ws_register(ctx->slab3, ctx->slab3_floats);
  }
  {
    const int widest = std::max({4 * R, 4 * Rq, K, M, S, A, Q});
    CK(dalloc(ctx, &ctx->coltmp3, (size_t)32 * widest));
    CK(dalloc(ctx, &ctx->coltmp2, (size_t)32 * widest));
    CK(dalloc(ctx, &ctx->dbi_part, (size_t)H * B * M));
    CK(dalloc(ctx, &ctx->tmpS, (size_t)S));
  }
  CK(dalloc(ctx, &ctx->dG1, TB * 4 * Rq));
  CK(dalloc(ctx, &ctx->dG2, TB * 4 * Rq));
  CK(dalloc(ctx, &ctx->dwe, TB * E));
  for (int L = 0; L < 2; ++L) {
    CK(dalloc(ctx, &ctx->edc[L][0], (size_t)B * Rq));
    CK(dalloc(ctx, &ctx->edc[L][1], (size_t)B * Rq));
  }
  CK(dalloc(ctx, &ctx->dkey, (size_t)2, false));
  CK(dalloc(ctx, &ctx->npart, (size_t)1024));
  CK(dalloc(ctx, &ctx->norms_d, (size_t)4));
#undef CK
  {
    hipError_t es = hipStreamSynchronize(ctx->st);
    if (es != hipSuccess) {
      rau_destroy(ctx);
      return fail(RAU_ERR_DEVICE, "rau_create sync: %s", hipGetErrorString(es));
    }
  }
  *out = ctx;
  return RAU_OK;
}

void rau_destroy(rau_ctx* ctx) {
  if (!ctx) return;
  rau_comm_destroy(ctx);
  if (ctx->st_comm) hipStreamDestroy(ctx->st_comm);
  if (ctx->evC) hipEventDestroy(ctx->evC);
  if (ctx->st) hipStreamSynchronize(ctx->st);
  if (ctx->st2) hipStreamSynchronize(ctx->st2);
  if (ctx->st3) hipStreamSynchronize(ctx->st3);
  for (auto& g : ctx->graphs) hipGraphExecDestroy(g.second);
  split_ws_unregister(ctx->slab);
  split_ws_unregister(ctx->slab2);
  split_ws_unregister(ctx->slab3);
  rau_bank_destroy(ctx);
  for (void* p : ctx->allocs) hipFree(p);
  if (ctx->hopw_h) hipHostFree(ctx->hopw_h);
  for (auto& r : ctx->precs) {
    hipEventDestroy(r.a);
    hipEventDestroy(r.b);
  }
  for (auto e : ctx->evpool) hipEventDestroy(e);
  if (ctx->ev0) hipEventDestroy(ctx->ev0);
  if (ctx->ev1) hipEventDestroy(ctx->ev1);
  for (hipEvent_t e : {ctx->evA, ctx->evD, ctx->evW, ctx->evE, ctx->evW3, ctx->evM3, ctx->evEnd, ctx->evE1,
                       ctx->evG0, ctx->evG, ctx->evQ0, ctx->evQ, ctx->evDq})
    if (e) hipEventDestroy(e);
  for (hipEvent_t e : ctx->evGc)
    if (e) hipEventDestroy(e);
  if (ctx->st3) hipStreamDestroy(ctx->st3);
  if (ctx->perr_h) hipHostFree(ctx->perr_h);
  if (ctx->stc) { hipStreamSynchronize(ctx->stc); hipStreamDestroy(ctx->stc); }
  for (BatchSlot& s : ctx->slot) {
    if (s.feats_h) hipHostFree(s.feats_h);
    if (s.image_of_h) hipHostFree(s.image_of_h);
    if (s.bank_idx_h) hipHostFree(s.bank_idx_h);
    if (s.uploaded) hipEventDestroy(s.uploaded);
    if (s.consumed) hipEventDestroy(s.consumed);
  }
  for (hipEvent_t e : ctx->hopw_ev) if (e) hipEventDestroy(e);
  for (hipEvent_t e : ctx->evF) hipEventDestroy(e);
  for (hipEvent_t e : ctx->evK) hipEventDestroy(e);

  for (hipEvent_t e : ctx->evH) hipEventDestroy(e);
  if (ctx->evHd) hipEventDestroy(ctx->evHd);
  if (ctx->st2) hipStreamDestroy(ctx->st2);
  if (ctx->st) hipStreamDestroy(ctx->st);
  delete ctx;
}

static int check_group(rau_ctx* ctx, int group) {
  NEED(ctx, "null ctx");
  NEED(group >= 0 && group < 3, "bad group %d", group);
  return 0;
}
int rau_params(rau_ctx* ctx, int group, float** weights, float** grads, size_t* n) {
  if (int rc = check_group(ctx, group)) return rc;
  if (weights) *weights = ctx->grp[group].w;
  if (grads) *grads = ctx->grp[group].g;
  if (n) *n = ctx->grp[group].n;
  return RAU_OK;
}
int rau_layout_count(const rau_ctx* ctx, int group) {
  if (!ctx || group < 0 || group > 2) return fail(RAU_ERR_INVALID, "bad ctx/group");
  return (int)ctx->grp[group].layout.size();
}
int rau_layout_entry(const rau_ctx* ctx, int group, int index, const char** name, size_t* offset,
                     int32_t* rows, int32_t* cols) {
  if (!ctx || group < 0 || group > 2) return fail(RAU_ERR_INVALID, "bad ctx/group");
  const auto& l = ctx->grp[group].layout;
  NEED(index >= 0 && index < (int)l.size(), "layout index %d out of range", index);
  if (name) *name = l[index].name.c_str();
  if (offset) *offset = l[index].off;
  if (rows) *rows = l[index].rows;
  if (cols) *cols = l[index].cols;
  return RAU_OK;
}
static int copy_group(rau_ctx* ctx, int group, bool grads, float* host, const float* chost,
                      size_t n) {
  if (int rc = check_group(ctx, group)) return rc;
  Group& g = ctx->grp[group];
  NEED(n == g.n, "group %d has %zu floats, caller passed %zu", group, g.n, n);
  float* dev = grads ? g.g : g.w;
  if (chost)
    HIPC(hipMemcpyAsync(dev, chost, n * sizeof(float), hipMemcpyHostToDevice, ctx->st));
  else
    HIPC(hipMemcpyAsync(host, dev, n * sizeof(float), hipMemcpyDeviceToHost, ctx->st));
  HIPC(hipStreamSynchronize(ctx->st));
  return RAU_OK;
}
int rau_set_params(rau_ctx* ctx, int group, const float* host, size_t n) {
  NEED(host, "null host pointer");
  return copy_group(ctx, group, false, nullptr, host, n);
}
int rau_get_params(rau_ctx* ctx, int group, float* host, size_t n) {
  NEED(host, "null host pointer");
  return copy_group(ctx, group, false, host, nullptr, n);
}
int rau_get_grads(rau_ctx* ctx, int group, float* host, size_t n) {
  NEED(host, "null host pointer");
  return copy_group(ctx, group, true, host, nullptr, n);
}
int rau_set_grads(rau_ctx* ctx, int group, const float* host, size_t n) {
  NEED(host, "null host pointer");
  return copy_group(ctx, group, true, nullptr, host, n);
}
int rau_init_uniform(rau_ctx* ctx, uint64_t seed, float lo, float hi) {
  NEED(ctx, "null ctx");
  for (int gi = 0; gi < 3; ++gi)
    RUN("uniform_fill", 0, ctx->grp[gi].n * 4.0,
        uniform_fill(ctx->st, seed, (uint32_t)gi, ctx->grp[gi].n, lo, hi, ctx->grp[gi].w));
  return RAU_OK;
}
int rau_zero_grads(rau_ctx* ctx) {
  NEED(ctx, "null ctx");
  for (int gi = 0; gi < 3; ++gi)
    HIPC(hipMemsetAsync(ctx->grp[gi].g, 0, ctx->grp[gi].n * sizeof(float), ctx->st));
  return RAU_OK;
}

int rau_set_mode(rau_ctx* ctx, int mode) {
  NEED(ctx, "null ctx");
  NEED(mode == RAU_MODE_TRAIN || mode == RAU_MODE_EVAL, "bad mode %d", mode);
  ctx->mode = mode;
  return RAU_OK;
}
int rau_set_dropout_seed(rau_ctx* ctx, uint64_t seed, uint32_t step) {
  NEED(ctx, "null ctx");
  ctx->seed = seed;
  ctx->step = step;
  for (int i = 0; i < 5; ++i) ctx->mexplicit[i] = false;
  ctx->mod_masks_valid = false;
  const uint64_t key[2] = {seed, (uint64_t)step};
  HIPC(hipMemcpyAsync(ctx->dkey, key, sizeof(key), hipMemcpyHostToDevice, ctx->st));
  return RAU_OK;
}
int rau_set_mask(rau_ctx* ctx, int site, const uint8_t* keep, size_t n) {
  NEED(ctx && keep, "null argument");
  NEED(site >= 0 && site < 5, "bad mask site %d", site);
  NEED(n == ctx->mcount[site], "mask site %d has %zu elements, caller passed %zu", site,
       ctx->mcount[site], n);
  std::vector<uint32_t> bits((n + 31) / 32, 0u);
  for (size_t i = 0; i < n; ++i)
    if (keep[i]) bits[i >> 5] |= 1u << (i & 31);
  HIPC(hipMemcpyAsync(ctx->mbits[site], bits.data(), bits.size() * 4, hipMemcpyHostToDevice,
                      ctx->st));
  HIPC(hipStreamSynchronize(ctx->st));
  ctx->mexplicit[site] = true;
  ctx->mod_masks_valid = false;
  return RAU_OK;
}
static int gen_masks(rau_ctx* ctx, int skip = -1, int only = -1, hipStream_t stream = nullptr) {
  if (ctx->mode != RAU_MODE_TRAIN) return 0;
  hipStream_t s = stream ? stream : ctx->st;
  for (int i = 0; i < 5; ++i)
    if (i != skip && (only < 0 || i == only) && !ctx->mexplicit[i] && ctx->mp[i] > 0.f)
      RUNS(s, "fill_masks", 0, ctx->mcount[i] / 8.0,
           fill_masks(s, ctx->seed, (uint32_t)i, ctx->step, ctx->mp[i], ctx->mcount[i],
                      ctx->mbits[i], ctx->dkey));
  return 0;
}
int rau_get_mask(rau_ctx* ctx, int site, uint8_t* keep, size_t n) {
  NEED(ctx && keep, "null argument");
  NEED(site >= 0 && site < 5, "bad mask site %d", site);
  NEED(n == ctx->mcount[site], "mask site %d has %zu elements, caller passed %zu", site,
       ctx->mcount[site], n);
  if (!ctx->mexplicit[site]) {
    const int m = ctx->mode;
    ctx->mode = RAU_MODE_TRAIN;
    const int rc = gen_masks(ctx);
    ctx->mode = m;
    if (rc) return rc;
  }
  std::vector<uint32_t> bits((n + 31) / 32);
  HIPC(hipMemcpyAsync(bits.data(), ctx->mbits[site], bits.size() * 4, hipMemcpyDeviceToHost,
                      ctx->st));
  HIPC(hipStreamSynchronize(ctx->st));
  for (size_t i = 0; i < n; ++i) keep[i] = (bits[i >> 5] >> (i & 31)) & 1u;
  return RAU_OK;
}

int rau_batch_size(rau_ctx* ctx, int32_t* n, int32_t* capacity) {
  NEED(ctx, "null ctx");
  if (n) *n = ctx->cfg.B;
  if (capacity) *capacity = ctx->cap;
  return RAU_OK;
}

namespace {
struct Regrow { float** ptr; size_t* have; size_t need; float* fresh; };
}
int rau_set_batch_size(rau_ctx* ctx, int32_t n) {
  NEED(ctx, "null ctx");
  NEED(n >= 1 && n <= ctx->cap, "rau_set_batch_size: n=%d out of [1,%d] (the B of rau_create)", n, ctx->cap);
  if (n == ctx->cfg.B) return RAU_OK;
  if (ctx->prof_on) return fail(RAU_ERR_STATE, "rau_set_batch_size: profiling must be off");
// ... 344 lines not shown
}

int rau_forward(rau_ctx* ctx) {
  NEED(ctx, "null ctx");
  BatchSlot& bs = cur_batch(ctx);
  if (!bs.held.have) return fail(RAU_ERR_STATE, "rau_forward: no batch (call rau_set_batch)");
  ctx->mg_valid = false;
  set_skinny_policy(ctx);
  const rau_config& c = ctx->cfg;
  const int B = c.B, E = c.E, Rq = c.Rq, D = c.D, S = ctx->Sp, SL = c.S, M = c.M, A = c.A, R = c.R,
            H = c.H, Q = ctx->Q;
  const int TL = bs.held.max_len;
  hipStream_t st = ctx->st;
  if (int rc = gen_masks(ctx, RAU_MASK_X)) return rc;
  const bool tr = ctx->mode == RAU_MODE_TRAIN;
  auto mk = [&](int site) -> const uint32_t* {
    return (tr && mask_p(ctx, site) > 0.f) ? ctx->mbits[site] : nullptr;
  };
  auto sc = [&](int site) { return 1.f / (1.f - mask_p(ctx, site)); };
  const uint32_t *m_we = mk(RAU_MASK_WE), *m_rnn = mk(RAU_MASK_RNN), *m_q = mk(RAU_MASK_Q),
                 *m_x = mk(RAU_MASK_X);
  const size_t BRq = (size_t)B * Rq;
  auto gflop = [](double m, double n, double k) { return 2.0 * m * n * k; };

  auto encoder_forward = [&]() -> int {
  if (TL > 0) {
    const int rows = TL * B;
    const size_t G4 = (size_t)B * 4 * Rq;
    RUN("embed_fwd", 0, rows * E * 8.0,
        embed_fwd(st, rows, E, c.V, ctx->grp[RAU_GROUP_EMBED].w, bs.tokens, m_we, sc(RAU_MASK_WE),
                  ctx->we));
    const bool ws_path = (ctx->mode == RAU_MODE_EVAL ? ctx->enc_ws : ctx->enc_ws_train) && ctx->perr_h;
    const int t_head = (!ws_path && side_split(ctx) && TL > kEncHeadTokens) ? kEncHeadTokens : TL;
    {
      LINOPTS(o);
      o.bias = ctx->i2h[0].b;
      o.bias2 = ctx->h2h[0].b;
      RUN("enc_i2h_gemm", gflop(t_head * B, 4 * Rq, E), 0,
          gemm_nt(st, t_head * B, 4 * Rq, E, ctx->we, E, ctx->i2h[0].W, E, ctx->G1, 4 * Rq, o));
    }
    if (t_head < TL) {
      HIPC(hipEventRecord(ctx->evG0, st));
      HIPC(hipStreamWaitEvent(ctx->st3, ctx->evG0, 0));
      LinOpts o;
      o.slab = ctx->slab3; o.slab_floats = ctx->slab3_floats;
      o.bias = ctx->i2h[0].b;
      o.bias2 = ctx->h2h[0].b;
      static const int nchunk_env = [] { const char* e = std::getenv("RAU_ENC_CHUNKS"); return e ? std::atoi(e) : 0; }();
      const int nchunk = std::max(1, std::min(nchunk_env > 0 ? nchunk_env : kEncSideChunks,
                                              std::min(kEncSideChunks, TL - t_head)));
      const int per = (TL - t_head + nchunk - 1) / nchunk;
      for (int cch = 0; cch <= kEncSideChunks; ++cch) ctx->enc_chunk_tok[cch] = TL;
      for (int cch = 0, t0 = t_head; t0 < TL; ++cch, t0 += per) {
        const int nt = std::min(per, TL - t0), r1 = nt * B;
        ctx->enc_chunk_tok[cch] = t0;
        RUNS(ctx->st3, "enc_i2h_gemm", gflop(r1, 4 * Rq, E), 0,
             gemm_nt(ctx->st3, r1, 4 * Rq, E, ctx->we + (size_t)t0 * B * E, E, ctx->i2h[0].W, E,
                     ctx->G1 + (size_t)t0 * G4, 4 * Rq, o));
        HIPC(hipEventRecord(ctx->evGc[cch], ctx->st3));
      }
    }
    auto wait_i2h_rows = [&](int s) -> int {
      if (t_head >= TL) return 0;
      for (int cch = 0; cch < kEncSideChunks; ++cch)
        if (ctx->enc_chunk_tok[cch] == s - 1 && s - 1 < TL) HIPC(hipStreamWaitEvent(st, ctx->evGc[cch], 0));
      return 0;
    };
    if (ws_path) {
      EncWsParams q{};
      q.B = B; q.R = Rq; q.TL = TL; q.bf16 = ctx->bf16 == 1;
      q.G1 = ctx->G1; q.G2 = ctx->G2; q.h1 = ctx->h1; q.c1 = ctx->c1; q.tc1 = ctx->tc1; q.x2 = ctx->x2;
      q.h2 = ctx->h2; q.c2 = ctx->c2; q.tc2 = ctx->tc2;
      q.Wh1 = ctx->h2h[0].W; q.Wi2 = ctx->i2h[1].W; q.Wh2 = ctx->h2h[1].W;
      q.bi2 = ctx->i2h[1].b; q.bh2 = ctx->h2h[1].b;
      q.mask = m_rnn; q.mscale = sc(RAU_MASK_RNN);
      q.cnt = ctx->ws_cnt; q.err = ctx->perr_d;
      RUN("enc_ws", (double)TL * 3 * gflop(B, 4 * Rq, Rq), 0, enc_ws_forward(st, GATES_DEEP, q));
      HIPC(hipMemcpyAsync(ctx->perr_h, ctx->perr_d, sizeof(int), hipMemcpyDeviceToHost, st));
      ctx->persist_used = true;
    } else
    for (int s = 1; s <= TL + 1; ++s) {
      if (int rc = wait_i2h_rows(s)) return rc;
      const float* Ap[3];
      const float* Wp[3];
      int nb = 0, i0 = -1, i1 = -1, i2 = -1;
      if (s <= TL && s >= 2) { Ap[nb] = ctx->h1 + (size_t)(s - 1) * BRq; Wp[nb] = ctx->h2h[0].W; i0 = nb++; }
      if (s >= 2) { Ap[nb] = ctx->x2 + (size_t)(s - 2) * BRq; Wp[nb] = ctx->i2h[1].W; i1 = nb++; }
      if (s >= 3) { Ap[nb] = ctx->h2 + (size_t)(s - 2) * BRq; Wp[nb] = ctx->h2h[1].W; i2 = nb++; }
      int nsp = 0;
      if (nb > 0)
        RUN("enc_h2h_gemm", gflop(B, 4 * Rq, Rq) * nb, 0,
            gemm_nt_batched_deferred(st, nb, B, 4 * Rq, Rq, Ap, Rq, Wp, Rq, ctx->slab,
                                     ctx->slab_floats, &nsp));
      LstmFwdCells cells{};
      if (s <= TL) {
        LstmFwdCell& C1 = cells.c[cells.n++];
        C1.g4 = ctx->G1 + (size_t)(s - 1) * G4;
        C1.has_input = 1;
        C1.slab = i0 >= 0 ? ctx->slab + (size_t)i0 * nsp * G4 : nullptr;
        C1.nsplit = i0 >= 0 ? nsp : 0;
        C1.c_prev = ctx->c1 + (size_t)(s - 1) * BRq; C1.cp_rs = Rq;
        C1.c = ctx->c1 + (size_t)s * BRq; C1.c_rs = Rq;
        C1.h = ctx->h1 + (size_t)s * BRq; C1.h_rs = Rq;
        C1.tanhc = ctx->tc1 + (size_t)(s - 1) * BRq;
        C1.drop_out = ctx->x2 + (size_t)(s - 1) * BRq;
        C1.mask = m_rnn; C1.mask_e0 = (size_t)(s - 1) * BRq; C1.mscale = sc(RAU_MASK_RNN);
      }
      if (s >= 2) {
        const int t = s - 1;
        LstmFwdCell& C2 = cells.c[cells.n++];
        C2.g4 = ctx->G2 + (size_t)(t - 1) * G4;
        C2.has_input = 0;
        C2.b1 = ctx->i2h[1].b; C2.b2 = ctx->h2h[1].b;
        C2.slab = ctx->slab + (size_t)i1 * nsp * G4;
        C2.nsplit = i2 >= 0 ? 2 * nsp : nsp;
        C2.c_prev = ctx->c2 + (size_t)(t - 1) * BRq; C2.cp_rs = Rq;
        C2.c = ctx->c2 + (size_t)t * BRq; C2.c_rs = Rq;
        C2.h = ctx->h2 + (size_t)t * BRq; C2.h_rs = Rq;
        C2.tanhc = ctx->tc2 + (size_t)(t - 1) * BRq;
        C2.drop_out = nullptr; C2.mask = nullptr; C2.mask_e0 = 0; C2.mscale = 1.f;
      }
      RUN("lstm_fwd", 0, BRq * 4.0 * 10 * cells.n, lstm_fwd_multi(st, GATES_DEEP, B, Rq, cells));
    }
  }
  return 0;
  };
  ctx->I_shared = (m_x == nullptr);
  const bool table_fwd = bs.held.n_images > 0 && ctx->I_shared && ctx->mode == RAU_MODE_EVAL && !ctx->capturing;
  const int nX = table_fwd ? bs.held.n_images : B;
  const int32_t* img = table_fwd ? bs.image_of_d : nullptr;
  const float* feats = bs.feats;
  if (table_fwd && bs.held.bank && !bs.held.table_ok) {
    const size_t map_bytes = (size_t)D * S * (bs.held.feat_type == RAU_FEAT_F32 ? 4 : 2);
    RUN("bank_gather", 0, 2.0 * nX * map_bytes,
        bank_gather(st, nX, map_bytes, ctx->bank, ctx->bank_cap, bs.bank_idx_d, bs.feats));
    bs.held.table_ok = true;
  }
  if (!table_fwd)
    if (int rc = batch_maps(ctx, &feats)) return rc;
  ctx->fwd_table = table_fwd;
  if (ctx->I_shared) {
    ctx->cur.assign(H, 0);
    ctx->cur[0] = H;
  } else {
    ctx->cur = ctx->groups;
  }
  const std::vector<int>& gsz = ctx->cur;
  {
    hipStream_t sb = ctx->st2;
    HIPC(hipEventRecord(ctx->evA, st));
    HIPC(hipStreamWaitEvent(sb, ctx->evA, 0));
    const bool x16 = m_x && ctx->xd16;
    const bool x_gen = m_x && !ctx->mexplicit[RAU_MASK_X] && SL == S && ((size_t)B * D * S) % 16 == 0;
    if (!x_gen)
      if (int rc = gen_masks(ctx, -1, RAU_MASK_X, sb)) return rc;
    RUNS(sb, "transpose", 0, (double)M * D * 8, transpose2d(sb, M, D, ctx->i_embed.W, ctx->WiT, ctx->WiT16));
    RUNS(sb, "transpose", 0, (double)A * M * 8, transpose2d(sb, A, M, ctx->att_i.W, ctx->WpT, ctx->WpT16));
    const int ft = bs.held.feat_type;
    const double xb = ft == RAU_FEAT_F32 ? 4 : 2;
    if (x_gen)
      RUNS(sb, "dropout_features", 0, (double)B * D * S * xb + (double)H * B * D * S * (x16 ? 2 : 4),
           dropout_features_gen(sb, ctx->seed, RAU_MASK_X, ctx->step, ctx->mp[RAU_MASK_X], ctx->dkey, H,
                                (size_t)B * D * S, feats, sc(RAU_MASK_X),
                                x16 ? (void*)ctx->xd16 : (void*)ctx->xd, x16 ? 1 : 0, ft));
    else if (x16)
      RUNS(sb, "dropout_features", 0, (double)B * D * S * xb + (double)H * B * D * S * 2,
           dropout_features_b16(sb, H, (size_t)B * D * S, feats, m_x, sc(RAU_MASK_X), ctx->xd16, ft));
    else if (m_x)
      RUNS(sb, "dropout_features", 0, (double)B * D * S * xb + (double)H * B * D * S * 4,
           dropout_features(sb, H, (size_t)B * D * S, feats, m_x, sc(RAU_MASK_X), ctx->xd, 0, SL,
                            S, ft));
    ctx->xw = const_cast<float*>(feats);
    if (!m_x && ft != RAU_FEAT_F32) {
      ctx->xw = ctx->xd;
      RUNS(sb, "widen_features", 0, (double)nX * D * S * (xb + 4),
           widen_features(sb, (size_t)nX * D, SL, S, feats, ctx->xw, ft));
    }
    for (int h0 = 0; h0 < H; h0 += gsz[h0]) {
      const int nBI = ctx->I_shared ? nX : gsz[h0] * B;
      const size_t hb = ctx->I_shared ? 0 : (size_t)h0 * B;
      const float* xin = m_x ? ctx->xd + hb * D * S : ctx->xw;
      float* Ig = ctx->I + hb * M * S;
      float* Pg = ctx->I_shared ? ctx->P0 : ctx->T + hb * A * S;
      if (x16)
        RUNS(sb, "conv_embed_fwd", gflop(M, (double)nBI * S, D),
             (double)nBI * D * S * 2 + (double)nBI * M * S * 4,
             conv_embed_fwd_b16(sb, nBI, D, S, M, (const uint16_t*)ctx->xd16 + hb * D * S, ctx->WiT16,
                                ctx->i_embed.b, Ig));
      else
        RUNS(sb, "conv_embed_fwd", gflop(M, (double)nBI * S, D),
             ((double)nBI * D * S + (double)nBI * M * S) * 4,
             conv_embed_fwd(sb, nBI, D, S, M, xin, ctx->WiT, ctx->i_embed.b, Ig, ctx->bf16));
      if (x16)
        RUNS(sb, "conv_att_pre", gflop(A, (double)nBI * S, M),
             ((double)nBI * M * S + (double)nBI * A * S) * 4,
             conv_att_pre_b16(sb, nBI, M, S, A, Ig, ctx->WpT16, ctx->att_i.b, Pg));
      else
        RUNS(sb, "conv_att_pre", gflop(A, (double)nBI * S, M),
             ((double)nBI * M * S + (double)nBI * A * S) * 4,
             conv_att_pre(sb, nBI, M, S, A, Ig, ctx->WpT, ctx->att_i.b, Pg, ctx->bf16));
      HIPC(hipEventRecord(ctx->evF[h0], sb));
    }
  }

  if (int rc = encoder_forward()) return rc;
  RUN("gather_q", 0, (double)B * Q * 8,
      gather_q(st, B, Rq, TL, bs.lens_d, ctx->c1, ctx->h1, ctx->c2, ctx->h2, ctx->q));

  const size_t BM_ = (size_t)B * M, BR_ = (size_t)B * R;
  RUN("apply_mask", 0, (double)H * B * Q * 8,
      apply_mask(st, (size_t)H * B * Q, (size_t)B * Q, ctx->q, m_q, sc(RAU_MASK_Q), ctx->qd));
  bool q_split = false;
  {
    ctx->yq_shared = (m_q == nullptr);
    q_split = !ctx->yq_shared && side_split(ctx) && H > 1;
    const int qrows = (ctx->yq_shared || q_split) ? B : H * B;
    LINOPTS(o);
    o.bias = ctx->q_proj.b;
    o.bias2 = ctx->h_proj.b;
    RUN("q_proj_gemm", gflop(qrows, M, Q), 0,
        gemm_nt(st, qrows, M, Q, ctx->qd, Q, ctx->q_proj.W, Q, ctx->Yq, M, o));
  }
  if (q_split) {
    HIPC(hipEventRecord(ctx->evQ0, st));
    HIPC(hipStreamWaitEvent(ctx->st3, ctx->evQ0, 0));
    LinOpts o;
    o.slab = ctx->slab3; o.slab_floats = ctx->slab3_floats;
    o.bias = ctx->q_proj.b;
    o.bias2 = ctx->h_proj.b;
    RUNS(ctx->st3, "q_proj_gemm", gflop((H - 1) * B, M, Q), 0,
         gemm_nt(ctx->st3, (H - 1) * B, M, Q, ctx->qd + (size_t)B * Q, Q, ctx->q_proj.W, Q,
                 ctx->Yq + (size_t)B * M, M, o));
    HIPC(hipEventRecord(ctx->evQ, ctx->st3));
  }
  HIPC(hipMemsetAsync(ctx->cc, 0, BR_ * sizeof(float), st));
  HIPC(hipMemsetAsync(ctx->hh, 0, BR_ * sizeof(float), st));
  const int32_t* labels = bs.held.have_labels ? bs.labels_d : nullptr;
  const size_t reg3 = ctx->slab3_floats / 4;
  const int head_max = (int)std::max<size_t>(1, reg3 / ((size_t)B * c.K));
  int gstart = 0;
  for (int h = 0; h < H; ++h) {
    if (gsz[h]) {
      HIPC(hipStreamWaitEvent(st, ctx->evF[h], 0));
      gstart = h;
    }
    if (h == 1 && q_split) HIPC(hipStreamWaitEvent(st, ctx->evQ, 0));
    if (int rc = hop_forward_chain(ctx, h, ctx->cc + (size_t)h * BR_, ctx->hh + (size_t)h * BR_,
                                   ctx->cc + (size_t)(h + 1) * BR_, ctx->hh + (size_t)(h + 1) * BR_,
                                   ctx->I + (ctx->I_shared ? 0 : (size_t)h * BM_ * S),
                                   ctx->I_shared ? ctx->P0 : ctx->T + (size_t)h * B * A * S, img))
      return rc;
    const bool group_end = h + 1 == H || gsz[h + 1] != 0;
    if (group_end || h + 1 - gstart >= head_max) {
      HIPC(hipEventRecord(ctx->evH[h], st));
      HIPC(hipStreamWaitEvent(ctx->st3, ctx->evH[h], 0));
      for (int h0 = gstart; h0 <= h; h0 += head_max)
        if (int rc = hop_forward_head(ctx, ctx->st3, ctx->slab3, reg3, h0,
                                      std::min(head_max, h + 1 - h0), labels))
          return rc;
      if (head_dgrad_fwd(ctx)) {
        const int nh = h + 1 - gstart;
        const bool trm = ctx->mode == RAU_MODE_TRAIN;
        LinOpts o;
        o.slab = ctx->slab3; o.slab_floats = ctx->slab3_floats;
        o.emask = (trm && mask_p(ctx, RAU_MASK_MF) > 0.f) ? ctx->mbits[RAU_MASK_MF] : nullptr;
        o.emask_e0 = (size_t)gstart * BM_;
        o.emscale = 1.f / (1.f - mask_p(ctx, RAU_MASK_MF));
        RUNS(ctx->st3, "head_dgrad", 2.0 * nh * B * M * c.K, 0,
             gemm_nn(ctx->st3, nh * B, M, c.K, ctx->dl + (size_t)gstart * B * c.K, c.K, ctx->cls.W, M,
                     ctx->dpre + (size_t)gstart * BM_, M, o));
        LinOpts o2;
        o2.slab = ctx->slab3; o2.slab_floats = ctx->slab3_floats;
        RUNS(ctx->st3, "head_dgrad", 2.0 * nh * B * R * M, 0,
             gemm_nn(ctx->st3, nh * B, R, M, ctx->dpre + (size_t)gstart * BM_, M, ctx->lstm_out.W, R,
                     ctx->dhn + (size_t)gstart * BR_, R, o2));
      }
      gstart = h + 1;
    }
  }
  HIPC(hipEventRecord(ctx->evHd, ctx->st3));
  HIPC(hipStreamWaitEvent(st, ctx->evHd, 0));
  if (bs.held.have_labels)
    RUN("loss_reduce", 0, 0, loss_reduce(st, H, B, ctx->lossrow, ctx->losses_d));
  if (!ctx->capturing) merge_record(ctx);
  ctx->fwd_done = true;
  ctx->dpre_fwd = head_dgrad_fwd(ctx);
  return RAU_OK;
}

static int upload_hop_weights(rau_ctx* ctx, const float* hop_w) {
  const int H = ctx->cfg.H;
  const int sl = (ctx->hopw_slot ^= 1);
  float* stage = ctx->hopw_h + (size_t)sl * H;
  if (!ctx->hopw_ev[sl]) HIPC(hipEventCreateWithFlags(&ctx->hopw_ev[sl], hipEventDisableTiming));
  else HIPC(hipEventSynchronize(ctx->hopw_ev[sl]));
  std::memcpy(stage, hop_w, (size_t)H * sizeof(float));
  HIPC(hipMemcpyAsync(ctx->hopw_d, stage, (size_t)H * sizeof(float), hipMemcpyHostToDevice, ctx->st));
  if (!ctx->capturing) HIPC(hipEventRecord(ctx->hopw_ev[sl], ctx->st));
  return 0;
}

int rau_backward(rau_ctx* ctx, const float* hop_w) {
  NEED(ctx && hop_w, "null argument");
  if (!ctx->fwd_done) return fail(RAU_ERR_STATE, "rau_backward: call rau_forward first");
  if (ctx->fwd_table)
    return fail(RAU_ERR_STATE, "rau_backward: the evaluate-mode forward of a batch with an image table computed "
                "i_embed once per image, so there is no per-sample I to differentiate; take evaluate-mode "
                "gradients on a plain batch (rau_set_batch)");
  set_skinny_policy(ctx);
  const BatchSlot& bs = cur_batch(ctx);
  if (!bs.held.have_labels) return fail(RAU_ERR_STATE, "rau_backward: batch has no labels");
  const rau_config& c = ctx->cfg;
  const int B = c.B, E = c.E, Rq = c.Rq, D = c.D, S = ctx->Sp, SL = c.S, M = c.M, A = c.A, R = c.R,
            K = c.K, H = c.H, Q = ctx->Q;
  const int TL = bs.held.max_len;
  std::vector<int> bsz_store;
  if (!ctx->I_shared && !ctx->bgroups.empty()) bsz_store = ctx->bgroups;
  const std::vector<int>& gsz = bsz_store.empty() ? ctx->cur : bsz_store;
  hipStream_t st = ctx->st;
  const bool tr = ctx->mode == RAU_MODE_TRAIN;
  auto mk = [&](int site) -> const uint32_t* {
    return (tr && mask_p(ctx, site) > 0.f) ? ctx->mbits[site] : nullptr;
  };
  auto sc = [&](int site) { return 1.f / (1.f - mask_p(ctx, site)); };
  const uint32_t *m_we = mk(RAU_MASK_WE), *m_rnn = mk(RAU_MASK_RNN), *m_q = mk(RAU_MASK_Q);
  auto gflop = [](double m, double n, double k) { return 2.0 * m * n * k; };
  const size_t BM_ = (size_t)B * M, BS_ = (size_t)B * S, BR_ = (size_t)B * R;
  const size_t BRq = (size_t)B * Rq;
  ctx->fwd_done = false;

  if (!ctx->capturing) {
    if (int rc = upload_hop_weights(ctx, hop_w)) return rc;
  }
  if (ctx->dpre_fwd)
    RUN("scale_hops", 0, (double)H * B * (K + M + R) * 8,
        scale_hops3(st, H, ctx->hopw_d, (size_t)B * K, ctx->dl, (size_t)B * M, ctx->dpre, (size_t)B * R, ctx->dhn));
  else
    RUN("scale_hops", 0, (double)H * B * K * 8, scale_hops(st, H, (size_t)B * K, ctx->hopw_d, ctx->dl));

  int HA = 0;
  for (int h = 0; h < H; ++h)
    if (hop_w[h] != 0.f) HA = h + 1;

  const uint32_t* m_mf = mk(RAU_MASK_MF);
  if (HA > 0 && !ctx->dpre_fwd) {
    LINOPTS(o);
    o.emask = m_mf;
    o.emask_e0 = 0;
    o.emscale = sc(RAU_MASK_MF);
    RUN("head_dgrad", gflop(HA * B, M, K), 0,
        gemm_nn(st, HA * B, M, K, ctx->dl, K, ctx->cls.W, M, ctx->dpre, M, o));
    LINOPTS(o2);
    RUN("head_dgrad", gflop(HA * B, R, M), 0,
        gemm_nn(st, HA * B, R, M, ctx->dpre, M, ctx->lstm_out.W, R, ctx->dhn, R, o2));
  }
  const float* dc_next = nullptr;
  float* dh_part = nullptr;
  int dh_part_ns = 0;
  ctx->ds16_step = ctx->dS16 && !ctx->I_shared && !ctx->att_split_env && conv_dz_fused_ok(S, M, ctx->bf16);
  struct Ds16Reset { rau_ctx* c; ~Ds16Reset() { c->ds16_step = false; } } ds16_reset{ctx};
  bool dq_side = false;
  int dq_rows_left = HA;
  for (int h = HA - 1; h >= 0; --h) {
    float* dc_out = ctx->dcn[h & 1];
    {
      HopGrad g{};
      g.dl = ctx->dl + (size_t)h * B * K;
      g.dc_next = dc_next;
      g.dh_next = nullptr;
      g.dc_out = dc_out;
      g.dh_out = nullptr;
      g.dpre_ready = 1;
      g.dhn_all = ctx->dhn;
      g.dh_part = dh_part;
      g.dh_part_ns = dh_part_ns;
      g.dh_part_out = &dh_part;
      g.dh_part_ns_out = &dh_part_ns;
      g.ev_conv_ready = (gsz[h] && (seam_mask() & 2)) ? ctx->evK[h] : nullptr;
      g.dh_prev_dead = h == 0;
      if (int rc = hop_backward(ctx, h, ctx->cc + (size_t)h * BR_,
                                ctx->I + (ctx->I_shared ? 0 : (size_t)h * BM_ * S), g))
        return rc;
    }
    dc_next = dc_out;
    if (gsz[h] && h > 0 && side_split(ctx)) {
      const int nh = std::min(h + gsz[h], HA) - h;
      HIPC(hipEventRecord(ctx->evK[h], st));
      HIPC(hipStreamWaitEvent(ctx->st3, ctx->evK[h], 0));
      LinOpts o;
      o.slab = ctx->slab3; o.slab_floats = ctx->slab3_floats;
      RUNS(ctx->st3, "q_proj_dgrad", gflop(nh * B, Q, M), 0,
           gemm_nn(ctx->st3, nh * B, Q, M, ctx->dqt + (size_t)h * BM_, M, ctx->q_proj.W, Q,
                   ctx->dQD + (size_t)h * B * Q, Q, o));
      HIPC(hipEventRecord(ctx->evDq, ctx->st3));
      dq_side = true;
      dq_rows_left = h;
    }
    if (gsz[h]) {
      hipStream_t sb = ctx->st2;
      if (!(seam_mask() & 2)) HIPC(hipEventRecord(ctx->evK[h], st));
      HIPC(hipStreamWaitEvent(sb, ctx->evK[h], 0));
      if (!ctx->I_shared) {
        const int nH = (std::min(h + gsz[h], HA) - h) * B;
        const size_t hb = (size_t)h * B;
        const int dzf = conv_dz_fused_ok(S, M, ctx->bf16);
        if (dzf)
          RUNS(sb, "conv_att_dgrad", gflop(M, (double)nH * S, A),
               ((double)nH * A * S + 3.0 * nH * M * S) * 4,
               conv_att_dgrad_dz(sb, nH, M, S, A,
                                 ctx->ds16_step ? (const float*)((const uint16_t*)ctx->dS16 + hb * A * S)
                                                : ctx->T + hb * A * S,
                                 ctx->att_i.W, ctx->dj + hb * M,
                                 ctx->a + hb * S, ctx->I + hb * M * S,
                                 ctx->xd16 ? (float*)((uint16_t*)ctx->dZ + hb * M * S) : ctx->dZ + hb * M * S,
                                 ctx->dbi_part + hb * M, ctx->xd16 ? 1 : 0, ctx->bf16, ctx->ds16_step ? 1 : 0,
                                 chain_bound(ctx) ? 1 : 0));
        else
          RUNS(sb, "conv_att_dgrad", gflop(M, (double)nH * S, A),
               ((double)nH * A * S + 2.0 * nH * M * S) * 4,
               conv_att_dgrad(sb, nH, M, S, A, ctx->T + hb * A * S, ctx->att_i.W, ctx->dj + hb * M,
                              ctx->a + hb * S, ctx->dZ + hb * M * S, ctx->bf16));
        {
          if (ctx->ds16_step)
            RUNS(sb, "conv_att_wgrad", gflop(A, M, (double)nH * S),
                 (double)nH * A * S * 2 + (double)nH * M * S * 4,
                 conv_att_wgrad_ds16(sb, nH, M, S, A, (const uint16_t*)ctx->dS16 + hb * A * S,
                                     ctx->I + hb * M * S, ctx->att_i.dW, ctx->slab2));
          else
          RUNS(sb, "conv_att_wgrad", gflop(A, M, (double)nH * S),
               ((double)nH * A * S + (double)nH * M * S) * 4,
               conv_att_wgrad(sb, nH, M, S, A, ctx->T + hb * A * S, ctx->I + hb * M * S,
                              ctx->att_i.dW, ctx->slab2, ctx->bf16));
        }
        if (ctx->xd16 && dzf)
          RUNS(sb, "conv_embed_wgrad", gflop(M, D, (double)nH * S),
               (double)nH * M * S * 2 + (double)nH * D * S * 2,
               conv_embed_wgrad_b16(sb, nH, D, S, M, (const uint16_t*)ctx->dZ + hb * M * S,
                                    (const uint16_t*)ctx->xd16 + hb * D * S, ctx->i_embed.dW, ctx->slab2));
        else
          RUNS(sb, "conv_embed_wgrad", gflop(M, D, (double)nH * S),
               ((double)nH * M * S * (dzf ? 1 : 2) + (double)nH * D * S) * 4,
               conv_embed_wgrad(sb, nH, D, S, M, ctx->dZ + hb * M * S, ctx->I + hb * M * S,
                                  ctx->xd + hb * D * S, ctx->i_embed.dW, ctx->slab2, ctx->bf16,
                                  ctx->i_embed.db, dzf));
        if (dzf && h == 0)
          RUNS(sb, "colsum", 0, (double)HA * B * M * 4,
               colsum_acc(sb, HA * B, M, ctx->dbi_part, M, ctx->i_embed.db, ctx->coltmp2));
      } else {
        for (int hh2 = 0; hh2 < HA; ++hh2) {
          float* Th2 = ctx->T + (size_t)hh2 * B * A * S;
          float* dZh = ctx->dZ + (size_t)hh2 * BM_ * S;
          RUNS(sb, "conv_att_dgrad", gflop(M, (double)B * S, A), ((double)B * A * S + 2.0 * BM_ * S) * 4,
               conv_att_dgrad(sb, B, M, S, A, Th2, ctx->att_i.W, ctx->dj + (size_t)hh2 * BM_,
                              ctx->a + (size_t)hh2 * BS_, dZh, ctx->bf16));
          RUNS(sb, "conv_att_wgrad", gflop(A, M, (double)B * S), ((double)B * A * S + BM_ * S) * 4,
               conv_att_wgrad(sb, B, M, S, A, Th2, ctx->I, ctx->att_i.dW, ctx->slab2, ctx->bf16));
          RUNS(sb, "conv_embed_wgrad", gflop(M, D, (double)B * S), (BM_ * S + (double)B * D * S) * 4,
               conv_embed_wgrad(sb, B, D, S, M, dZh, ctx->I, ctx->xw, ctx->i_embed.dW, ctx->slab2,
                                ctx->bf16, ctx->i_embed.db));
        }
      }
    }
  }
  {
    LINOPTS(o);
    if (dq_rows_left > 0)
      RUN("q_proj_dgrad", gflop(dq_rows_left * B, Q, M), 0,
          gemm_nn(st, dq_rows_left * B, Q, M, ctx->dqt, M, ctx->q_proj.W, Q, ctx->dQD, Q, o));
    if (dq_side) HIPC(hipStreamWaitEvent(st, ctx->evDq, 0));
    RUN("dq_reduce", 0, (double)HA * B * Q * 4,
        dq_reduce(st, HA, (size_t)B * Q, ctx->dQD, m_q, sc(RAU_MASK_Q), ctx->dq));
  }
  {
    hipStream_t sb = ctx->st2;
    HIPC(hipEventRecord(ctx->evD, sb));
  }
  HIPC(hipEventRecord(ctx->evW, st));
  static const int wg_env = [] { const char* e = std::getenv("RAU_WG_BULK"); return e ? std::atoi(e) : -1; }();
  const int wg_bulk = side_split(ctx) ? 0 : wg_env >= 0 ? wg_env : (chain_bound(ctx) ? 0 : 1);
  auto mult_wgrads = [&]() -> int {
    hipStream_t sw = (wg_bulk & 1) ? ctx->st2 : ctx->st3;
    HIPC(hipStreamWaitEvent(sw, ctx->evW, 0));
    const int rows = HA * B;
    if (rows == 0) {
      HIPC(hipEventRecord(ctx->evM3, sw));
      return 0;
    }
    {
      TnProblem pr[13];
      const int np = mult_wgrad_problems(ctx, pr);
      double fl = 0;
      for (int i = 0; i < np; ++i) fl += gflop(pr[i].M, pr[i].N, rows);
      float* ws = (wg_bulk & 1) ? ctx->slab2 : ctx->slab3;
      const size_t ws_floats = (wg_bulk & 1) ? ctx->slab2_floats : ctx->slab3_floats;
      RUNS(sw, "wgrad_gemm", fl, 0, gemm_tn_group_acc(sw, pr, np, rows, ws, ws_floats, ctx->bf16 == 1));
    }
    float* ct = (wg_bulk & 1) ? ctx->coltmp2 : ctx->coltmp3;
    RUNS(sw, "colsum", 0, (double)rows * A * 4, colsum_acc(sw, rows, A, ctx->dwsp, A, ctx->att_score.dW, ct));
    HIPC(hipMemsetAsync(ctx->tmpS, 0, S * sizeof(float), sw));
    RUNS(sw, "colsum", 0, (double)rows * S * 4, colsum_acc(sw, rows, SL, ctx->dz, S, ctx->tmpS, ct));
    RUNS(sw, "colsum", 0, S * 4.0, colsum_acc(sw, SL, 1, ctx->tmpS, 1, ctx->att_score.db, ct));
    RUNS(sw, "colsum", 0, (double)rows * A * 4, colsum_acc(sw, rows, A, ctx->du, A, ctx->att_i.db, ct));
    HIPC(hipEventRecord(ctx->evM3, sw));
    return 0;
  };
  if (int rc = mult_wgrads()) return rc;

  if (TL > 0) {
    const int rows = TL * B;
    const size_t G4 = (size_t)B * 4 * Rq;
    auto enc_wgrads = [&](int t_lo, int t_hi, hipEvent_t ev) -> int {
      if (t_hi <= t_lo) return 0;
      hipStream_t sw = (wg_bulk & 2) ? ctx->st2 : ctx->st3;
      HIPC(hipEventRecord(ev, st));
      HIPC(hipStreamWaitEvent(sw, ev, 0));
      const size_t r0 = (size_t)t_lo * B;
      const int nr = (t_hi - t_lo) * B;
      TnProblem pr[13];
      const int np = enc_wgrad_problems(ctx, r0, pr);
      double fl = 0;
      for (int i = 0; i < np; ++i) fl += gflop(pr[i].M, pr[i].N, nr);
      float* ws = (wg_bulk & 2) ? ctx->slab2 : ctx->slab3;
      const size_t ws_floats = (wg_bulk & 2) ? ctx->slab2_floats : ctx->slab3_floats;
      RUNS(sw, "wgrad_gemm", fl, 0, gemm_tn_group_acc(sw, pr, np, nr, ws, ws_floats, ctx->bf16 == 1));
      return 0;
    };
    const int hi = TL;
    for (int u = TL; u >= 0; --u) {
      const float* Ap[3];
      const float* Wp[3];
      int nb = 0, iq2 = -1, iqx = -1, iq1 = -1;
      if (u >= 1 && u + 1 <= TL) { Ap[nb] = ctx->dG2 + (size_t)u * G4; Wp[nb] = ctx->h2h[1].W; iq2 = nb++; }
      if (u + 1 <= TL) { Ap[nb] = ctx->dG2 + (size_t)u * G4; Wp[nb] = ctx->i2h[1].W; iqx = nb++; }
      if (u + 2 <= TL) { Ap[nb] = ctx->dG1 + (size_t)(u + 1) * G4; Wp[nb] = ctx->h2h[0].W; iq1 = nb++; }
      int nsp = 0;
      if (nb > 0)
        RUN("enc_h2h_dgrad", gflop(B, Rq, 4 * Rq) * nb, 0,
            gemm_nn_batched_deferred(st, nb, B, Rq, 4 * Rq, Ap, 4 * Rq, Wp, Rq, ctx->slab,
                                     ctx->slab_floats, &nsp));
      LstmBwdCells cells{};
      cells.lens = bs.lens_d;
      cells.dq_rs = Q;
      if (u >= 1) {
        LstmBwdCell& C2 = cells.c[cells.n++];
        C2.gates = ctx->G2 + (size_t)(u - 1) * G4;
        C2.c_prev = ctx->c2 + (size_t)(u - 1) * BRq; C2.cp_rs = Rq;
        C2.tanhc = ctx->tc2 + (size_t)(u - 1) * BRq;
        C2.slabA = iq2 >= 0 ? ctx->slab + (size_t)iq2 * nsp * BRq : nullptr;
        C2.nA = iq2 >= 0 ? nsp : 0;
        C2.slabB = nullptr; C2.nBp = 0; C2.maskB = nullptr; C2.maskB_e0 = 0; C2.mscaleB = 1.f;
        C2.dc_next = u < TL ? ctx->edc[1][(u + 1) & 1] : nullptr;
        C2.dsum = ctx->dG2 + (size_t)(u - 1) * G4;
        C2.dc_prev = ctx->edc[1][u & 1];
        C2.t = u; C2.dq_c = ctx->dq + 2 * Rq; C2.dq_h = ctx->dq + 3 * Rq;
      }
      if (u + 1 <= TL) {
        const int t = u + 1;
        LstmBwdCell& C1 = cells.c[cells.n++];
        C1.gates = ctx->G1 + (size_t)u * G4;
        C1.c_prev = ctx->c1 + (size_t)u * BRq; C1.cp_rs = Rq;
        C1.tanhc = ctx->tc1 + (size_t)u * BRq;
        C1.slabA = iq1 >= 0 ? ctx->slab + (size_t)iq1 * nsp * BRq : nullptr;
        C1.nA = iq1 >= 0 ? nsp : 0;
        C1.slabB = ctx->slab + (size_t)iqx * nsp * BRq;
        C1.nBp = nsp;
        C1.maskB = m_rnn; C1.maskB_e0 = (size_t)u * BRq; C1.mscaleB = sc(RAU_MASK_RNN);
        C1.dc_next = t < TL ? ctx->edc[0][(t + 1) & 1] : nullptr;
        C1.dsum = ctx->dG1 + (size_t)u * G4;
        C1.dc_prev = ctx->edc[0][t & 1];
        C1.t = t; C1.dq_c = ctx->dq; C1.dq_h = ctx->dq + Rq;
      }
      RUN("lstm_bwd", 0, BRq * 4.0 * 12 * cells.n, lstm_bwd_multi(st, GATES_DEEP, B, Rq, cells));
    }
    {
      LINOPTS(o);
      RUN("enc_i2h_dgrad", gflop(rows, E, 4 * Rq), 0,
          gemm_nn(st, rows, E, 4 * Rq, ctx->dG1, 4 * Rq, ctx->i2h[0].W, E, ctx->dwe, E, o));
    }
    RUN("embed_bwd", 0, (double)rows * E * 12,
        embed_bwd(st, ctx->capturing ? c.T * B : bs.held.nuniq, E, bs.utok, bs.ustart, bs.upos, ctx->dwe, ctx->we, m_we,
                  sc(RAU_MASK_WE), ctx->grp[RAU_GROUP_EMBED].g));
    if (int rc = enc_wgrads(0, hi, ctx->evE)) return rc;
  }
  HIPC(hipEventRecord(ctx->evW3, ctx->st3));
  HIPC(hipStreamWaitEvent(st, ctx->evW3, 0));
  if (wg_bulk) HIPC(hipEventRecord(ctx->evD, ctx->st2));
  HIPC(hipStreamWaitEvent(st, ctx->evD, 0));
  HIPC(hipEventRecord(ctx->evEnd, st));
  ctx->bwd_done = true;
  ctx->graph_last = false;
  return RAU_OK;
}

int rau_graph_step(rau_ctx* ctx, const float* hop_w, int zero_grads_first) {
  NEED(ctx && hop_w, "null argument");
  const BatchSlot& bs = cur_batch(ctx);
  if (!bs.held.have || !bs.held.have_labels)
    return fail(RAU_ERR_STATE, "rau_graph_step: needs a batch with labels (rau_set_batch)");
  if (ctx->prof_on) return fail(RAU_ERR_STATE, "rau_graph_step: profiling must be off");
  const int H = ctx->cfg.H;
  int HA = 0;
  for (int h = 0; h < H; ++h)
    if (hop_w[h] != 0.f) HA = h + 1;
  uint64_t key = (uint64_t)ctx->mode | ((uint64_t)bs.held.max_len << 2) | ((uint64_t)HA << 12) |
                 ((uint64_t)(zero_grads_first != 0) << 22);
  for (int i = 0; i < 5; ++i) key |= (uint64_t)ctx->mexplicit[i] << (24 + i);
  key |= (uint64_t)ctx->cur_slot << 30;
  key |= (uint64_t)bs.held.feat_type << 32;
  key |= (uint64_t)(bs.held.n_images > 0) << 34;
  key |= (uint64_t)bs.held.bank << 35;
  key |= (uint64_t)ctx->cfg.B << 36;
  if (int rc = upload_hop_weights(ctx, hop_w)) return rc;
  ctx->mg_valid = false;
  hipGraphExec_t exec = nullptr;
  for (auto& g : ctx->graphs)
    if (g.first == key) exec = g.second;
  if (!exec) {
    hipGraph_t graph = nullptr;
    HIPC(hipStreamBeginCapture(ctx->st, hipStreamCaptureModeRelaxed));
    ctx->capturing = true;
    int rc = zero_grads_first ? rau_zero_grads(ctx) : 0;
    if (!rc) rc = rau_forward(ctx);
    if (!rc) rc = rau_backward(ctx, hop_w);
    ctx->capturing = false;
    hipError_t e = hipStreamEndCapture(ctx->st, &graph);
    if (rc) {
      if (graph) hipGraphDestroy(graph);
      return rc;
    }
    if (e != hipSuccess)
      return fail(RAU_ERR_DEVICE, "hipStreamEndCapture: %s", hipGetErrorString(e));
    e = hipGraphInstantiate(&exec, graph, nullptr, nullptr, 0);
    hipGraphDestroy(graph);
    if (e != hipSuccess)
      return fail(RAU_ERR_DEVICE, "hipGraphInstantiate: %s", hipGetErrorString(e));
    ctx->graphs.push_back({key, exec});
  }
  HIPC(hipGraphLaunch(exec, ctx->st));
  if (bs.held.n_images) {
    ctx->x_valid = true;
    ctx->x_slot = ctx->cur_slot;
    ctx->x_serial = ctx->slot_serial[ctx->cur_slot];
  }
  HIPC(hipEventRecord(ctx->evEnd, ctx->st));
  merge_record(ctx);
  ctx->fwd_done = false;
  ctx->bwd_done = true;
  ctx->graph_last = true;
  return RAU_OK;
}
// ... 251 lines not shown
```

### rau_vqa_amd/csrc/wgrad_dma.hip

```cpp
#include <type_traits>
#include <utility>

#include "common.h"
#include "kernels.h"

namespace rau {

namespace {

constexpr int GS = 196;
constexpr int GCH = 28;
constexpr int GNCH = GS / GCH;
constexpr int GT = 128;
constexpr int GPART = GT * GCH;
constexpr int GSTAGE = 2 * GPART;
constexpr int GNST = 2;

typedef __attribute__((address_space(3))) void* lds_ptr_t;
typedef const __attribute__((address_space(1))) void* glb_ptr_t;

struct WgradParams {
  int ra, rb, nB, tiles_a, tiles_b, splits, spb;
  const float* A; long a_bs;
  const float* B; long b_bs;
  float* slab;
};

template <class F, int... I>
__device__ __forceinline__ void gfor_impl(F&& f, std::integer_sequence<int, I...>) {
  (f(std::integral_constant<int, I>{}), ...);
}
template <int N, class F>
__device__ __forceinline__ void gfor(F&& f) { gfor_impl(f, std::make_integer_sequence<int, N>{}); }

template <int OFF>
__device__ __forceinline__ void lds_read64(float2& dst, uint32_t addr) {
  asm volatile("ds_read_b64 %0, %1 offset:%2" : "=v"(dst) : "v"(addr), "n"(OFF) : "memory");
}
template <int OFF>
__device__ __forceinline__ void lds_read32(float& dst, uint32_t addr) {
  asm volatile("ds_read_b32 %0, %1 offset:%2" : "=v"(dst) : "v"(addr), "n"(OFF) : "memory");
}

template <int NG>
__global__ __launch_bounds__(256 * NG, 2) void k_wgrad_dma(const WgradParams P) {
  __shared__ __attribute__((aligned(16))) float smem_all[NG * GNST * GSTAGE];
  const int tid = threadIdx.x, l = tid & 63;
  const int wv = __builtin_amdgcn_readfirstlane(tid >> 6);
  const int grp = NG == 1 ? 0 : wv >> 2;
  const int w = wv & 3;
  float* smem = smem_all + grp * (GNST * GSTAGE);
  const int wm = w & 1, wn = w >> 1;
  const int tiles = P.tiles_a * P.tiles_b;
  const int L = blockIdx.x, r8 = L & 7, q8 = L >> 3;
  const int split = r8 + 8 * (q8 / tiles), tile = q8 % tiles;
  if (split >= P.splits) return;
  const int ta = tile % P.tiles_a, tb = tile / P.tiles_a;
  const int b_lo = split * P.spb;
  int b_hi = b_lo + P.spb;
  if (b_hi > P.nB) b_hi = P.nB;
  const int nst_all = (b_hi - b_lo) * GNCH;
  const int nst = (nst_all - grp + NG - 1) / NG;
  const int nloop = (nst_all + NG - 1) / NG;

  uint32_t voff[7];
#pragma unroll
  for (int n = 0; n < 7; ++n) {
    const int i = w + 4 * n;
    const int p = 64 * (i < 14 ? i : i - 14) + l;
    voff[n] = (uint32_t)((p / 7) * GS * 4 + (p % 7) * 16);
  }
  const char* a0 = reinterpret_cast<const char*>(P.A + (size_t)b_lo * P.a_bs + (size_t)ta * GT * GS);
  const char* b0 = reinterpret_cast<const char*>(P.B + (size_t)b_lo * P.b_bs + (size_t)tb * GT * GS);
  const char *ap = nullptr, *bp = nullptr;
  float* dst = nullptr;
  auto stage_ptrs = [&](int sg) {
    const int s = NG * sg + grp;
    const int sb = s / GNCH, ch = s - sb * GNCH;
    ap = a0 + ((size_t)sb * P.a_bs + ch * GCH) * 4;
    bp = b0 + ((size_t)sb * P.b_bs + ch * GCH) * 4;
    dst = smem + (sg & 1) * GSTAGE;
  };
  auto issue_slot = [&](int n) {
    const int i = w + 4 * n;
    uint32_t vo = voff[n];
    asm volatile("" : "+v"(vo));
    __builtin_amdgcn_global_load_lds((glb_ptr_t)((i < 14 ? ap : bp) + vo),
                                     (lds_ptr_t)(dst + (i < 14 ? 0 : GPART) + 256 * (i < 14 ? i : i - 14)),
                                     16, 0, 0);
  };

  f32x4 acc[4][4];
#pragma unroll
  for (int i = 0; i < 4; ++i)
#pragma unroll
    for (int j = 0; j < 4; ++j) acc[i][j] = f32x4{0.f, 0.f, 0.f, 0.f};

  const int row = l & 15, g = l >> 4;
  const uint32_t lds0 = (uint32_t)(size_t)(lds_ptr_t)smem;
  const uint32_t fa64 = lds0 + (uint32_t)((wm * 64 + row) * GCH + 2 * g) * 4;
  const uint32_t fb64 = lds0 + (uint32_t)(GPART + (wn * 64 + row) * GCH + 2 * g) * 4;
  const uint32_t fa32 = lds0 + (uint32_t)((wm * 64 + row) * GCH + 24 + g) * 4;
  const uint32_t fb32 = lds0 + (uint32_t)(GPART + (wn * 64 + row) * GCH + 24 + g) * 4;
  constexpr int BLK = 16 * GCH * 4;

  if (nst > 0) {
    stage_ptrs(0);
#pragma unroll
    for (int n = 0; n < 7; ++n) issue_slot(n);
  }
#pragma unroll 1
  for (int s = 0; s < nloop; ++s) {
    asm volatile("s_waitcnt vmcnt(0)" ::: "memory");
    __builtin_amdgcn_s_barrier();
    if (NG > 1 && s >= nst) continue;
    const bool more = s + 1 < nst;
    if (more) stage_ptrs(s + 1);
    const uint32_t so = (uint32_t)((s & 1) * GSTAGE) * 4;
    float2 a2[2][4], b2[2][4];
    float a1[4], b1[4];
    auto rd64 = [&](auto kk_tag, int set) {
      constexpr int KK = decltype(kk_tag)::value;
      gfor<4>([&](auto it) {
        constexpr int i = decltype(it)::value;
        lds_read64<i * BLK + KK * 32>(a2[set][i], fa64 + so);
        lds_read64<i * BLK + KK * 32>(b2[set][i], fb64 + so);
      });
    };
    auto mma64 = [&](int set, int slot) {
#pragma unroll
      for (int i = 0; i < 4; ++i)
#pragma unroll
        for (int j = 0; j < 4; ++j)
          acc[i][j] = __builtin_amdgcn_mfma_f32_16x16x4f32(a2[set][i].x, b2[set][j].x, acc[i][j], 0, 0, 0);
      if (more) issue_slot(slot);
#pragma unroll
      for (int i = 0; i < 4; ++i)
#pragma unroll
        for (int j = 0; j < 4; ++j)
          acc[i][j] = __builtin_amdgcn_mfma_f32_16x16x4f32(a2[set][i].y, b2[set][j].y, acc[i][j], 0, 0, 0);
      if (more) issue_slot(slot + 1);
    };
    using K0 = std::integral_constant<int, 0>;
    using K1 = std::integral_constant<int, 1>;
    using K2 = std::integral_constant<int, 2>;
    rd64(K0{}, 0);
    rd64(K1{}, 1);
    asm volatile("s_waitcnt lgkmcnt(8)" ::: "memory");
    __builtin_amdgcn_sched_barrier(0);
    mma64(0, 0);
    __builtin_amdgcn_sched_barrier(0);
    rd64(K2{}, 0);
    asm volatile("s_waitcnt lgkmcnt(8)" ::: "memory");
    __builtin_amdgcn_sched_barrier(0);
    mma64(1, 2);
    __builtin_amdgcn_sched_barrier(0);
    gfor<4>([&](auto it) {
      constexpr int i = decltype(it)::value;
      lds_read32<i * BLK>(a1[i], fa32 + so);
      lds_read32<i * BLK>(b1[i], fb32 + so);
    });
    asm volatile("s_waitcnt lgkmcnt(8)" ::: "memory");
    __builtin_amdgcn_sched_barrier(0);
    mma64(0, 4);
    __builtin_amdgcn_sched_barrier(0);
    asm volatile("s_waitcnt lgkmcnt(0)" ::: "memory");
    __builtin_amdgcn_sched_barrier(0);
#pragma unroll
    for (int i = 0; i < 4; ++i)
#pragma unroll
      for (int j = 0; j < 4; ++j)
        acc[i][j] = __builtin_amdgcn_mfma_f32_16x16x4f32(a1[i], b1[j], acc[i][j], 0, 0, 0);
    if (more) issue_slot(6);
    __builtin_amdgcn_sched_barrier(0);
  }

  if (NG > 1) {
    static_assert(NG == 1 || (size_t)4 * 16 * 64 * 16 <= (size_t)NG * GNST * GSTAGE * 4, "exchange area fits");
    __builtin_amdgcn_s_barrier();
    f32x4* xch = reinterpret_cast<f32x4*>(smem_all);
    if (grp == 1) {
#pragma unroll
      for (int i = 0; i < 4; ++i)
#pragma unroll
        for (int j = 0; j < 4; ++j) xch[((w * 16 + i * 4 + j) << 6) + l] = acc[i][j];
    }
    __syncthreads();
    if (grp == 1) return;
#pragma unroll
    for (int i = 0; i < 4; ++i)
#pragma unroll
      for (int j = 0; j < 4; ++j) {
        const f32x4 o = xch[((w * 16 + i * 4 + j) << 6) + l];
        acc[i][j][0] += o[0]; acc[i][j][1] += o[1]; acc[i][j][2] += o[2]; acc[i][j][3] += o[3];
      }
  }
  float* C = P.slab + (size_t)split * P.ra * P.rb;
#pragma unroll
  for (int i = 0; i < 4; ++i)
#pragma unroll
    for (int j = 0; j < 4; ++j) {
      const int cb = tb * GT + wn * 64 + j * 16 + row;
#pragma unroll
      for (int r = 0; r < 4; ++r) {
        const int ca = ta * GT + wm * 64 + i * 16 + 4 * g + r;
        C[(size_t)ca * P.rb + cb] = acc[i][j][r];
      }
    }
}

}

bool wgrad_dma_ok(int ra, int rb, int S) {
  static const bool off = std::getenv("RAU_WGRAD_DMA_OFF") != nullptr;
  return !off && S == GS && ra % GT == 0 && rb % GT == 0;
}

hipError_t wgrad_dma(hipStream_t st, int nB, int ra, int rb, int S, const float* A, long a_bs,
                     const float* B, long b_bs, float* dW, float* slab, int splits) {
  if (!wgrad_dma_ok(ra, rb, S) || nB < 1 || splits < 1) return hipErrorInvalidValue;
  WgradParams P{};
  P.ra = ra; P.rb = rb; P.nB = nB;
  P.tiles_a = ra / GT; P.tiles_b = rb / GT;
  P.spb = (nB + splits - 1) / splits;
  P.splits = (nB + P.spb - 1) / P.spb;
  P.A = A; P.a_bs = a_bs; P.B = B; P.b_bs = b_bs; P.slab = slab;
  static const int genv = [] { const char* e = std::getenv("RAU_WGRAD_GROUPS"); return e ? std::atoi(e) : 0; }();
  const int groups = genv == 1 || genv == 2 ? genv : (P.tiles_a * P.tiles_b <= 8 ? 2 : 1);
  if (groups == 2 && splits >= 2) {
    const int s2 = (splits + 1) / 2;
    P.spb = (nB + s2 - 1) / s2;
    P.splits = (nB + P.spb - 1) / P.spb;
    const dim3 grid(8 * ((P.splits + 7) / 8) * P.tiles_a * P.tiles_b);
    hipLaunchKernelGGL(k_wgrad_dma<2>, grid, dim3(512), 0, st, P);
  } else {
    const dim3 grid(8 * ((P.splits + 7) / 8) * P.tiles_a * P.tiles_b);
    hipLaunchKernelGGL(k_wgrad_dma<1>, grid, dim3(256), 0, st, P);
  }
  hipError_t e = hipGetLastError();
  if (e != hipSuccess) return e;
  return splitk_reduce_acc(st, (size_t)ra * rb, P.splits, slab, (size_t)ra * rb, dW);
}

}
```

Baseline: 27620 QA-pairs/s.

## Defer conv wgrad split-k reductions to side stream and split feature dropout per hop group

Conv attention and embedding weight-gradient kernels now accumulate into persistent per-split slabs across hop groups, using a fixed split plan. A single split-k reduction per weight runs on a side stream after the last group, replacing one reduction per group on the main stream. Feature dropout for later hop groups is generated on a side stream with per-group events, so the first conv can start sooner. The bias colsum and tail colsums also move to the side stream. This costs extra slab workspace, read-modify-write accumulation in the wgrad epilogue, and added event synchronisation.

```diff
diff --git a/rau_vqa_amd/csrc/gemm_conv.hip b/rau_vqa_amd/csrc/gemm_conv.hip
--- a/rau_vqa_amd/csrc/gemm_conv.hip
+++ b/rau_vqa_amd/csrc/gemm_conv.hip
@@ -140,7 +140,7 @@
   return launch_gemm<128, 128, BK, SRC_RC, SRC_RC_FLAT, EPI_CONV>(st, P, 1);
 }
 
-static int conv_wgrad_splits(int nB, int rowsA, int rowsB) {
+int conv_wgrad_splits(int nB, int rowsA, int rowsB) {
   const int tiles = ((rowsA + 127) / 128) * ((rowsB + 127) / 128);
   constexpr int target = 512;
   int s = target / tiles;
diff --git a/rau_vqa_amd/csrc/kernels.h b/rau_vqa_amd/csrc/kernels.h
--- a/rau_vqa_amd/csrc/kernels.h
+++ b/rau_vqa_amd/csrc/kernels.h
@@ -115,6 +115,11 @@
 bool wgrad_dma_ok(int ra, int rb, int S);
 hipError_t wgrad_dma(hipStream_t st, int nB, int ra, int rb, int S, const float* A, long a_bs,
                      const float* B, long b_bs, float* dW, float* slab, int splits);
+int conv_wgrad_splits(int nB, int rowsA, int rowsB);
+int wgrad_dma_plan(int nB_max, int ra, int rb, int splits);
+hipError_t wgrad_dma_partial(hipStream_t st, int nB, int ra, int rb, int S, const float* A, long a_bs,
+                             const float* B, long b_bs, float* slab, int splits, int plan, int accumulate);
+hipError_t wgrad_dma_reduce(hipStream_t st, int ra, int rb, const float* slab, int plan, float* dW);
 hipError_t conv_att_wgrad(hipStream_t st, int nB, int M, int S, int A, const float* dS,
                           const float* I, float* dWp, float* slab, int bf16 = 0);
 hipError_t conv_embed_wgrad(hipStream_t st, int nB, int D, int S, int M, const float* dI,
@@ -207,7 +212,7 @@
                             const uint32_t* mask, float mscale, float* xd, size_t mask_e0 = 0,
                             int SL = 0, int Sp = 0, int ft = RAU_FEAT_F32);
 hipError_t dropout_features_gen(hipStream_t st, uint64_t seed, uint32_t site, uint32_t step, float p,
-                                const uint64_t* key_dev, int H, size_t per_hop, const void* X,
+                                const uint64_t* key_dev, int h0, int nh, size_t per_hop, const void* X,
                                 float mscale, void* xd, int b16, int ft = RAU_FEAT_F32);
 hipError_t dropout_features_b16(hipStream_t st, int H, size_t per_hop, const void* X,
                                 const uint32_t* mask, float mscale, void* xd16, int ft = RAU_FEAT_F32);
diff --git a/rau_vqa_amd/csrc/kernels.hip b/rau_vqa_amd/csrc/kernels.hip
--- a/rau_vqa_amd/csrc/kernels.hip
+++ b/rau_vqa_amd/csrc/kernels.hip
@@ -1369,7 +1369,7 @@
 }
 template <bool B16, int FT>
 __global__ void k_dropout_features_gen(uint64_t seed, uint32_t site, uint32_t step, uint32_t thr,
-                                       const uint64_t* __restrict__ key, int H, size_t per16,
+                                       const uint64_t* __restrict__ key, int h0, int nh, size_t per16,
                                        const void* __restrict__ X, float mscale,
                                        void* __restrict__ xd) {
   if (key) {
@@ -1388,7 +1388,7 @@
       x[r] = ok[r] ? load_feat4<FT>(X, 4 * blk + quad) : make_float4(0.f, 0.f, 0.f, 0.f);
     }
     const size_t mine = base + l < per16 ? base + l : per16 - 1;
-    for (int h = 0; h < H; ++h) {
+    for (int h = h0; h < h0 + nh; ++h) {
       const uint32_t bits = philox_keep16(seed, site, step, (size_t)h * per16 + mine, thr);
 #pragma unroll
       for (int r = 0; r < 4; ++r) {
@@ -1414,29 +1414,29 @@
 }
 template <bool B16>
 static void launch_dropout_gen(hipStream_t st, int ft, dim3 grid, uint64_t seed, uint32_t site,
-                               uint32_t step, uint32_t thr, const uint64_t* key, int H, size_t per16,
+                               uint32_t step, uint32_t thr, const uint64_t* key, int h0, int nh, size_t per16,
                                const void* X, float mscale, void* xd) {
   if (ft == RAU_FEAT_F16)
     hipLaunchKernelGGL((k_dropout_features_gen<B16, RAU_FEAT_F16>), grid, dim3(256), 0, st, seed, site, step,
-                       thr, key, H, per16, X, mscale, xd);
+                       thr, key, h0, nh, per16, X, mscale, xd);
   else if (ft == RAU_FEAT_BF16)
     hipLaunchKernelGGL((k_dropout_features_gen<B16, RAU_FEAT_BF16>), grid, dim3(256), 0, st, seed, site, step,
-                       thr, key, H, per16, X, mscale, xd);
+                       thr, key, h0, nh, per16, X, mscale, xd);
   else
     hipLaunchKernelGGL((k_dropout_features_gen<B16, RAU_FEAT_F32>), grid, dim3(256), 0, st, seed, site, step,
-                       thr, key, H, per16, X, mscale, xd);
+                       thr, key, h0, nh, per16, X, mscale, xd);
 }
 hipError_t dropout_features_gen(hipStream_t st, uint64_t seed, uint32_t site, uint32_t step, float p,
-                                const uint64_t* key_dev, int H, size_t per_hop, const void* X,
+                                const uint64_t* key_dev, int h0, int nh, size_t per_hop, const void* X,
                                 float mscale, void* xd, int b16, int ft) {
-  if (per_hop % 16 != 0 || !feat_type_ok(ft)) return hipErrorInvalidValue;
+  if (per_hop % 16 != 0 || !feat_type_ok(ft) || h0 < 0 || nh < 1) return hipErrorInvalidValue;
   const uint32_t thr = (uint32_t)lroundf(p * 256.0f);
   const size_t per16 = per_hop / 16;
   if (b16)
-    launch_dropout_gen<true>(st, ft, dim3(grid_for(per16)), seed, site, step, thr, key_dev, H, per16, X,
+    launch_dropout_gen<true>(st, ft, dim3(grid_for(per16)), seed, site, step, thr, key_dev, h0, nh, per16, X,
                              mscale, xd);
   else
-    launch_dropout_gen<false>(st, ft, dim3(grid_for(per16)), seed, site, step, thr, key_dev, H, per16, X,
+    launch_dropout_gen<false>(st, ft, dim3(grid_for(per16)), seed, site, step, thr, key_dev, h0, nh, per16, X,
                               mscale, xd);
   return hipGetLastError();
 }
diff --git a/rau_vqa_amd/csrc/rau_ctx.h b/rau_vqa_amd/csrc/rau_ctx.h
--- a/rau_vqa_amd/csrc/rau_ctx.h
+++ b/rau_vqa_amd/csrc/rau_ctx.h
@@ -104,6 +104,8 @@
   int enc_chunk_tok[kEncSideChunks + 1] = {};
   std::vector<hipEvent_t> evH;
   std::vector<hipEvent_t> evF, evK;
+  std::vector<hipEvent_t> evX;
+  hipEvent_t evDg = nullptr, evRa = nullptr, evRe = nullptr;
   std::vector<int> groups, cur, bgroups;
   std::vector<void*> allocs;
   std::vector<std::pair<void*, size_t>> scratch;
@@ -169,6 +171,7 @@
   float *dpre, *dhn, *dg4, *dcn[2], *dhp[2], *dj, *da_lin, *dz, *du, *dwsp, *dZ,
       *dqt, *dQD, *dq, *slab, *slab2, *slab3, *coltmp3, *tmpS, *coltmp2, *dbi_part;
   size_t slab3_floats = 0, slab2_floats = 0;
+  size_t wstep_off = 0, wstep_emb = 0;
   size_t slab_alloc = 0, slab2_alloc = 0, slab3_alloc = 0;
   float *dG1, *dG2, *dwe, *edc[2][2];
   size_t slab_floats = 0;
diff --git a/rau_vqa_amd/csrc/rau_ctx.hip b/rau_vqa_amd/csrc/rau_ctx.hip
--- a/rau_vqa_amd/csrc/rau_ctx.hip
+++ b/rau_vqa_amd/csrc/rau_ctx.hip
@@ -69,6 +69,7 @@
   std::vector<int> groups;
   bool att_split, enc_ws, enc_ws_train;
   size_t slab, slab2, slab3, att_part;
+  size_t wstep_off, wstep_emb;
   size_t mcount[5];
 };
 static void plan_batch(rau_ctx* ctx, int B, BatchPlan* p) {
@@ -130,7 +131,9 @@
       for (int tt = 1; tt <= T; ++tt)
         grp_floats = std::max(grp_floats, gemm_tn_group_slab_floats(pr, n, tt * B));
     }
-    p->slab2 = std::max(sl2, grp_floats);
+    p->wstep_off = (std::max(sl2, grp_floats) + 3) / 4 * 4;
+    p->wstep_emb = p->wstep_off + (conv_wgrad_slab_floats(H * B, A, M, S) + 3) / 4 * 4;
+    p->slab2 = p->wstep_emb + conv_wgrad_slab_floats(H * B, M, D, S);
     const int rowsH = H * B, rowsT = T * B;
     const int shapes[][3] = {{K, M, rowsH},      {M, R, rowsH},      {4 * R, M, rowsH},
                              {4 * R, R, rowsH},  {M, S, rowsH},      {S, R, rowsH},
@@ -150,6 +153,8 @@
   ctx->enc_ws_train = p.enc_ws_train;
   ctx->slab_floats = p.slab;
   ctx->slab2_floats = p.slab2;
+  ctx->wstep_off = p.wstep_off;
+  ctx->wstep_emb = p.wstep_emb;
   ctx->slab3_floats = p.slab3;
 }
 
@@ -257,7 +262,7 @@
   hipEventCreate(&ctx->ev1);
   const unsigned evflags = hipEventDisableTiming;
   for (hipEvent_t* e : {&ctx->evA, &ctx->evD, &ctx->evW, &ctx->evE, &ctx->evW3, &ctx->evM3, &ctx->evEnd, &ctx->evE1,
-                        &ctx->evG0, &ctx->evG, &ctx->evQ0, &ctx->evQ, &ctx->evDq})
+                        &ctx->evG0, &ctx->evG, &ctx->evQ0, &ctx->evQ, &ctx->evDq, &ctx->evDg, &ctx->evRa, &ctx->evRe})
     hipEventCreateWithFlags(e, evflags);
   for (hipEvent_t& e : ctx->evGc) hipEventCreateWithFlags(&e, evflags);
   {
@@ -287,12 +292,12 @@
   }
   ctx->evF.resize(c.H);
   ctx->evK.resize(c.H);
-
+  ctx->evX.resize(c.H);
   ctx->evH.resize(c.H);
   for (int i = 0; i < c.H; ++i) {
     hipEventCreateWithFlags(&ctx->evF[i], evflags);
     hipEventCreateWithFlags(&ctx->evK[i], evflags);
-
+    hipEventCreateWithFlags(&ctx->evX[i], evflags);
     hipEventCreateWithFlags(&ctx->evH[i], evflags);
   }
   hipEventCreateWithFlags(&ctx->evHd, evflags);
@@ -510,7 +515,7 @@
   if (ctx->ev0) hipEventDestroy(ctx->ev0);
   if (ctx->ev1) hipEventDestroy(ctx->ev1);
   for (hipEvent_t e : {ctx->evA, ctx->evD, ctx->evW, ctx->evE, ctx->evW3, ctx->evM3, ctx->evEnd, ctx->evE1,
-                       ctx->evG0, ctx->evG, ctx->evQ0, ctx->evQ, ctx->evDq})
+                       ctx->evG0, ctx->evG, ctx->evQ0, ctx->evQ, ctx->evDq, ctx->evDg, ctx->evRa, ctx->evRe})
     if (e) hipEventDestroy(e);
   for (hipEvent_t e : ctx->evGc)
     if (e) hipEventDestroy(e);
@@ -527,7 +532,7 @@
   for (hipEvent_t e : ctx->hopw_ev) if (e) hipEventDestroy(e);
   for (hipEvent_t e : ctx->evF) hipEventDestroy(e);
   for (hipEvent_t e : ctx->evK) hipEventDestroy(e);
-
+  for (hipEvent_t e : ctx->evX) hipEventDestroy(e);
   for (hipEvent_t e : ctx->evH) hipEventDestroy(e);
   if (ctx->evHd) hipEventDestroy(ctx->evHd);
   if (ctx->st2) hipStreamDestroy(ctx->st2);
@@ -1178,17 +1183,31 @@
     HIPC(hipStreamWaitEvent(sb, ctx->evA, 0));
     const bool x16 = m_x && ctx->xd16;
     const bool x_gen = m_x && !ctx->mexplicit[RAU_MASK_X] && SL == S && ((size_t)B * D * S) % 16 == 0;
+    bool x_split = false;
     if (!x_gen)
       if (int rc = gen_masks(ctx, -1, RAU_MASK_X, sb)) return rc;
     RUNS(sb, "transpose", 0, (double)M * D * 8, transpose2d(sb, M, D, ctx->i_embed.W, ctx->WiT, ctx->WiT16));
     RUNS(sb, "transpose", 0, (double)A * M * 8, transpose2d(sb, A, M, ctx->att_i.W, ctx->WpT, ctx->WpT16));
     const int ft = bs.held.feat_type;
     const double xb = ft == RAU_FEAT_F32 ? 4 : 2;
-    if (x_gen)
-      RUNS(sb, "dropout_features", 0, (double)B * D * S * xb + (double)H * B * D * S * (x16 ? 2 : 4),
-           dropout_features_gen(sb, ctx->seed, RAU_MASK_X, ctx->step, ctx->mp[RAU_MASK_X], ctx->dkey, H,
+    x_split = x_gen && !x16 && !ctx->bf16 && gsz[0] < H;
+    if (x_gen) {
+      const int nh0 = x_split ? gsz[0] : H;
+      RUNS(sb, "dropout_features", 0, (double)B * D * S * xb + (double)nh0 * B * D * S * (x16 ? 2 : 4),
+           dropout_features_gen(sb, ctx->seed, RAU_MASK_X, ctx->step, ctx->mp[RAU_MASK_X], ctx->dkey, 0, nh0,
                                 (size_t)B * D * S, feats, sc(RAU_MASK_X),
                                 x16 ? (void*)ctx->xd16 : (void*)ctx->xd, x16 ? 1 : 0, ft));
+      if (x_split) {
+        hipStream_t sw = ctx->st3;
+        HIPC(hipStreamWaitEvent(sw, ctx->evA, 0));
+        for (int h0 = gsz[0]; h0 < H; h0 += gsz[h0]) {
+          RUNS(sw, "dropout_features", 0, (double)B * D * S * xb + (double)gsz[h0] * B * D * S * 4,
+               dropout_features_gen(sw, ctx->seed, RAU_MASK_X, ctx->step, ctx->mp[RAU_MASK_X], ctx->dkey, h0,
+                                    gsz[h0], (size_t)B * D * S, feats, sc(RAU_MASK_X), (void*)ctx->xd, 0, ft));
+          HIPC(hipEventRecord(ctx->evX[h0], sw));
+        }
+      }
+    }
     else if (x16)
       RUNS(sb, "dropout_features", 0, (double)B * D * S * xb + (double)H * B * D * S * 2,
            dropout_features_b16(sb, H, (size_t)B * D * S, feats, m_x, sc(RAU_MASK_X), ctx->xd16, ft));
@@ -1208,6 +1227,7 @@
       const float* xin = m_x ? ctx->xd + hb * D * S : ctx->xw;
       float* Ig = ctx->I + hb * M * S;
       float* Pg = ctx->I_shared ? ctx->P0 : ctx->T + hb * A * S;
+      if (x_split && h0 > 0) HIPC(hipStreamWaitEvent(sb, ctx->evX[h0], 0));
       if (x16)
         RUNS(sb, "conv_embed_fwd", gflop(M, (double)nBI * S, D),
              (double)nBI * D * S * 2 + (double)nBI * M * S * 4,
@@ -1387,6 +1407,24 @@
   struct Ds16Reset { rau_ctx* c; ~Ds16Reset() { c->ds16_step = false; } } ds16_reset{ctx};
   bool dq_side = false;
   int dq_rows_left = HA;
+  static const int wg_env = [] { const char* e = std::getenv("RAU_WG_BULK"); return e ? std::atoi(e) : -1; }();
+  const int wg_bulk = side_split(ctx) ? 0 : wg_env >= 0 ? wg_env : (chain_bound(ctx) ? 0 : 1);
+  const bool dzf_step = conv_dz_fused_ok(S, M, ctx->bf16);
+  const bool tail_side = (wg_bulk & 1) && !ctx->I_shared;
+  const bool wstep = (wg_bulk & 1) && !ctx->I_shared && !ctx->bf16 && !ctx->ds16_step && dzf_step && !ctx->xd16 &&
+                     wgrad_dma_ok(A, M, S) && wgrad_dma_ok(M, D, S);
+  int nB_max = 0;
+  for (int h = 0; h < HA; ++h)
+    if (gsz[h]) nB_max = std::max(nB_max, (std::min(h + gsz[h], HA) - h) * B);
+  const int plan_att = wstep && nB_max ? wgrad_dma_plan(nB_max, A, M, conv_wgrad_splits(nB_max, A, M)) : 0;
+  const int plan_emb = wstep && nB_max ? wgrad_dma_plan(nB_max, M, D, conv_wgrad_splits(nB_max, M, D)) : 0;
+  float* const slab_att = ctx->slab2 + ctx->wstep_off;
+  float* const slab_emb = ctx->slab2 + ctx->wstep_emb;
+  if (wstep && nB_max &&
+      ((size_t)plan_att * A * M > ctx->wstep_emb - ctx->wstep_off ||
+       (size_t)plan_emb * M * D > ctx->slab2_floats - ctx->wstep_emb))
+    return fail(RAU_ERR_STATE, "rau_backward: the conv weight gradients' split plan exceeds its workspace");
+  bool wstep_first = true;
   for (int h = HA - 1; h >= 0; --h) {
     float* dc_out = ctx->dcn[h & 1];
     {
@@ -1446,30 +1484,60 @@
                ((double)nH * A * S + 2.0 * nH * M * S) * 4,
                conv_att_dgrad(sb, nH, M, S, A, ctx->T + hb * A * S, ctx->att_i.W, ctx->dj + hb * M,
                               ctx->a + hb * S, ctx->dZ + hb * M * S, ctx->bf16));
+        if (dzf && h == 0 && tail_side) {
+          HIPC(hipEventRecord(ctx->evDg, sb));
+          HIPC(hipStreamWaitEvent(ctx->st3, ctx->evDg, 0));
+          RUNS(ctx->st3, "colsum", 0, (double)HA * B * M * 4,
+               colsum_acc(ctx->st3, HA * B, M, ctx->dbi_part, M, ctx->i_embed.db, ctx->coltmp3));
+        }
         {
           if (ctx->ds16_step)
             RUNS(sb, "conv_att_wgrad", gflop(A, M, (double)nH * S),
                  (double)nH * A * S * 2 + (double)nH * M * S * 4,
                  conv_att_wgrad_ds16(sb, nH, M, S, A, (const uint16_t*)ctx->dS16 + hb * A * S,
                                      ctx->I + hb * M * S, ctx->att_i.dW, ctx->slab2));
+          else if (wstep)
+            RUNS(sb, "conv_att_wgrad", gflop(A, M, (double)nH * S),
+                 ((double)nH * A * S + (double)nH * M * S) * 4,
+                 wgrad_dma_partial(sb, nH, A, M, S, ctx->T + hb * A * S, (long)A * S, ctx->I + hb * M * S,
+                                   (long)M * S, slab_att, conv_wgrad_splits(nH, A, M), plan_att,
+                                   wstep_first ? 0 : 1));
           else
           RUNS(sb, "conv_att_wgrad", gflop(A, M, (double)nH * S),
                ((double)nH * A * S + (double)nH * M * S) * 4,
                conv_att_wgrad(sb, nH, M, S, A, ctx->T + hb * A * S, ctx->I + hb * M * S,
                               ctx->att_i.dW, ctx->slab2, ctx->bf16));
+          if (wstep && h == 0) {
+            HIPC(hipEventRecord(ctx->evRa, sb));
+            HIPC(hipStreamWaitEvent(ctx->st3, ctx->evRa, 0));
+            RUNS(ctx->st3, "splitk_reduce", 0, (double)(plan_att + 2) * A * M * 4,
+                 wgrad_dma_reduce(ctx->st3, A, M, slab_att, plan_att, ctx->att_i.dW));
+          }
         }
         if (ctx->xd16 && dzf)
           RUNS(sb, "conv_embed_wgrad", gflop(M, D, (double)nH * S),
                (double)nH * M * S * 2 + (double)nH * D * S * 2,
                conv_embed_wgrad_b16(sb, nH, D, S, M, (const uint16_t*)ctx->dZ + hb * M * S,
                                     (const uint16_t*)ctx->xd16 + hb * D * S, ctx->i_embed.dW, ctx->slab2));
-        else
+        else if (wstep) {
+          RUNS(sb, "conv_embed_wgrad", gflop(M, D, (double)nH * S), ((double)nH * M * S + (double)nH * D * S) * 4,
+               wgrad_dma_partial(sb, nH, M, D, S, ctx->dZ + hb * M * S, (long)M * S, ctx->xd + hb * D * S,
+                                 (long)D * S, slab_emb, conv_wgrad_splits(nH, M, D), plan_emb,
+                                 wstep_first ? 0 : 1));
+          wstep_first = false;
+          if (h == 0) {
+            HIPC(hipEventRecord(ctx->evRe, sb));
+            HIPC(hipStreamWaitEvent(ctx->st3, ctx->evRe, 0));
+            RUNS(ctx->st3, "splitk_reduce", 0, (double)(plan_emb + 2) * M * D * 4,
+                 wgrad_dma_reduce(ctx->st3, M, D, slab_emb, plan_emb, ctx->i_embed.dW));
+          }
+        } else
           RUNS(sb, "conv_embed_wgrad", gflop(M, D, (double)nH * S),
                ((double)nH * M * S * (dzf ? 1 : 2) + (double)nH * D * S) * 4,
                conv_embed_wgrad(sb, nH, D, S, M, ctx->dZ + hb * M * S, ctx->I + hb * M * S,
                                   ctx->xd + hb * D * S, ctx->i_embed.dW, ctx->slab2, ctx->bf16,
                                   ctx->i_embed.db, dzf));
-        if (dzf && h == 0)
+        if (dzf && h == 0 && !tail_side)
           RUNS(sb, "colsum", 0, (double)HA * B * M * 4,
                colsum_acc(sb, HA * B, M, ctx->dbi_part, M, ctx->i_embed.db, ctx->coltmp2));
       } else {
@@ -1502,8 +1570,6 @@
     HIPC(hipEventRecord(ctx->evD, sb));
   }
   HIPC(hipEventRecord(ctx->evW, st));
-  static const int wg_env = [] { const char* e = std::getenv("RAU_WG_BULK"); return e ? std::atoi(e) : -1; }();
-  const int wg_bulk = side_split(ctx) ? 0 : wg_env >= 0 ? wg_env : (chain_bound(ctx) ? 0 : 1);
   auto mult_wgrads = [&]() -> int {
     hipStream_t sw = (wg_bulk & 1) ? ctx->st2 : ctx->st3;
     HIPC(hipStreamWaitEvent(sw, ctx->evW, 0));
@@ -1518,10 +1584,14 @@
       double fl = 0;
       for (int i = 0; i < np; ++i) fl += gflop(pr[i].M, pr[i].N, rows);
       float* ws = (wg_bulk & 1) ? ctx->slab2 : ctx->slab3;
-      const size_t ws_floats = (wg_bulk & 1) ? ctx->slab2_floats : ctx->slab3_floats;
+      const size_t ws_floats = (wg_bulk & 1) ? ctx->wstep_off : ctx->slab3_floats;
       RUNS(sw, "wgrad_gemm", fl, 0, gemm_tn_group_acc(sw, pr, np, rows, ws, ws_floats, ctx->bf16 == 1));
     }
-    float* ct = (wg_bulk & 1) ? ctx->coltmp2 : ctx->coltmp3;
+    if (tail_side) {
+      sw = ctx->st3;
+      HIPC(hipStreamWaitEvent(sw, ctx->evW, 0));
+    }
+    float* ct = sw == ctx->st2 ? ctx->coltmp2 : ctx->coltmp3;
     RUNS(sw, "colsum", 0, (double)rows * A * 4, colsum_acc(sw, rows, A, ctx->dwsp, A, ctx->att_score.dW, ct));
     HIPC(hipMemsetAsync(ctx->tmpS, 0, S * sizeof(float), sw));
     RUNS(sw, "colsum", 0, (double)rows * S * 4, colsum_acc(sw, rows, SL, ctx->dz, S, ctx->tmpS, ct));
diff --git a/rau_vqa_amd/csrc/wgrad_dma.hip b/rau_vqa_amd/csrc/wgrad_dma.hip
--- a/rau_vqa_amd/csrc/wgrad_dma.hip
+++ b/rau_vqa_amd/csrc/wgrad_dma.hip
@@ -24,6 +24,7 @@
   const float* A; long a_bs;
   const float* B; long b_bs;
   float* slab;
+  int accumulate;
 };
 
 template <class F, int... I>
@@ -59,6 +60,10 @@
   const int b_lo = split * P.spb;
   int b_hi = b_lo + P.spb;
   if (b_hi > P.nB) b_hi = P.nB;
+  if (b_hi <= b_lo) {
+    if (P.accumulate) return;
+    b_hi = b_lo;
+  }
   const int nst_all = (b_hi - b_lo) * GNCH;
   const int nst = (nst_all - grp + NG - 1) / NG;
   const int nloop = (nst_all + NG - 1) / NG;
@@ -204,7 +209,8 @@
 #pragma unroll
       for (int r = 0; r < 4; ++r) {
         const int ca = ta * GT + wm * 64 + i * 16 + 4 * g + r;
-        C[(size_t)ca * P.rb + cb] = acc[i][j][r];
+        float* c = C + (size_t)ca * P.rb + cb;
+        *c = P.accumulate ? *c + acc[i][j][r] : acc[i][j][r];
       }
     }
 }
@@ -216,30 +222,58 @@
   return !off && S == GS && ra % GT == 0 && rb % GT == 0;
 }
 
-hipError_t wgrad_dma(hipStream_t st, int nB, int ra, int rb, int S, const float* A, long a_bs,
-                     const float* B, long b_bs, float* dW, float* slab, int splits) {
-  if (!wgrad_dma_ok(ra, rb, S) || nB < 1 || splits < 1) return hipErrorInvalidValue;
+static int wgrad_groups(int ra, int rb, int splits) {
+  static const int genv = [] { const char* e = std::getenv("RAU_WGRAD_GROUPS"); return e ? std::atoi(e) : 0; }();
+  const int groups = genv == 1 || genv == 2 ? genv : ((ra / GT) * (rb / GT) <= 8 ? 2 : 1);
+  return groups == 2 && splits >= 2 ? 2 : 1;
+}
+static int wgrad_splits(int nB, int ra, int rb, int splits) {
+  if (wgrad_groups(ra, rb, splits) == 2) splits = (splits + 1) / 2;
+  const int spb = (nB + splits - 1) / splits;
+  return (nB + spb - 1) / spb;
+}
+int wgrad_dma_plan(int nB_max, int ra, int rb, int splits) { return wgrad_splits(nB_max, ra, rb, splits); }
+
+static hipError_t wgrad_launch(hipStream_t st, int nB, int ra, int rb, int S, const float* A, long a_bs,
+                               const float* B, long b_bs, float* slab, int splits, int plan, int accumulate,
+                               int* used) {
+  if (!wgrad_dma_ok(ra, rb, S) || nB < 1 || splits < 1 || plan < 0) return hipErrorInvalidValue;
   WgradParams P{};
   P.ra = ra; P.rb = rb; P.nB = nB;
   P.tiles_a = ra / GT; P.tiles_b = rb / GT;
-  P.spb = (nB + splits - 1) / splits;
-  P.splits = (nB + P.spb - 1) / P.spb;
-  P.A = A; P.a_bs = a_bs; P.B = B; P.b_bs = b_bs; P.slab = slab;
-  static const int genv = [] { const char* e = std::getenv("RAU_WGRAD_GROUPS"); return e ? std::atoi(e) : 0; }();
-  const int groups = genv == 1 || genv == 2 ? genv : (P.tiles_a * P.tiles_b <= 8 ? 2 : 1);
-  if (groups == 2 && splits >= 2) {
-    const int s2 = (splits + 1) / 2;
-    P.spb = (nB + s2 - 1) / s2;
-    P.splits = (nB + P.spb - 1) / P.spb;
-    const dim3 grid(8 * ((P.splits + 7) / 8) * P.tiles_a * P.tiles_b);
+  const int groups = wgrad_groups(ra, rb, splits);
+  if (plan) {
+    P.splits = plan;
+    P.spb = (nB + plan - 1) / plan;
+  } else {
+    P.splits = wgrad_splits(nB, ra, rb, splits);
+    P.spb = (nB + P.splits - 1) / P.splits;
+  }
+  P.A = A; P.a_bs = a_bs; P.B = B; P.b_bs = b_bs; P.slab = slab; P.accumulate = accumulate;
+  if (used) *used = P.splits;
+  const dim3 grid(8 * ((P.splits + 7) / 8) * P.tiles_a * P.tiles_b);
+  if (groups == 2)
     hipLaunchKernelGGL(k_wgrad_dma<2>, grid, dim3(512), 0, st, P);
-  } else {
-    const dim3 grid(8 * ((P.splits + 7) / 8) * P.tiles_a * P.tiles_b);
+  else
     hipLaunchKernelGGL(k_wgrad_dma<1>, grid, dim3(256), 0, st, P);
-  }
-  hipError_t e = hipGetLastError();
+  return hipGetLastError();
+}
+
+hipError_t wgrad_dma(hipStream_t st, int nB, int ra, int rb, int S, const float* A, long a_bs,
+                     const float* B, long b_bs, float* dW, float* slab, int splits) {
+  int used = 0;
+  hipError_t e = wgrad_launch(st, nB, ra, rb, S, A, a_bs, B, b_bs, slab, splits, 0, 0, &used);
   if (e != hipSuccess) return e;
-  return splitk_reduce_acc(st, (size_t)ra * rb, P.splits, slab, (size_t)ra * rb, dW);
-}
-
-}
+  return splitk_reduce_acc(st, (size_t)ra * rb, used, slab, (size_t)ra * rb, dW);
+}
+
+hipError_t wgrad_dma_partial(hipStream_t st, int nB, int ra, int rb, int S, const float* A, long a_bs,
+                             const float* B, long b_bs, float* slab, int splits, int plan, int accumulate) {
+  if (plan < 1 || !split_span_ok(slab, plan, (size_t)ra * rb)) return plan < 1 ? hipErrorInvalidValue : kSplitStateError;
+  return wgrad_launch(st, nB, ra, rb, S, A, a_bs, B, b_bs, slab, splits, plan, accumulate, nullptr);
+}
+hipError_t wgrad_dma_reduce(hipStream_t st, int ra, int rb, const float* slab, int plan, float* dW) {
+  return splitk_reduce_acc(st, (size_t)ra * rb, plan, slab, (size_t)ra * rb, dW);
+}
+
+}
```

Result: slower. 26970 QA-pairs/s (-2.3%).
